# deepmarkpy/aware

Hardware: AMD Instinct MI355X
Metric: waveform-seconds/sec through embed->attack->detect; BER vs reference (higher is better)
Workload: dtype f32 accumulation on the 16-bit MFMA pipe; conv-block GEMMs: every f32 operand scaled by a power of two and carried as TWO binary16 terms (within one f32 ulp of the operand, rms 2^-24.5), 3 partial products, the l_a*l_b term (<= 2^-22) dropped -- gemm_h2.hip: error level of an f32 dot product (agains

## Files before the change

### aware_amd/_lib.py

```python
from __future__ import annotations

import ctypes as C
import glob
import os
import subprocess

_HERE = os.path.dirname(os.path.abspath(__file__))
LIB_PATH = os.environ.get("AWARE_HIP_LIB") or os.path.join(_HERE, "libaware_hip.so")
CSRC = os.path.join(_HERE, "csrc")
SOURCES = ["capi.hip", "dsp_kernels.hip", "dsp_stream.hip", "seam_kernels.hip", "detector_kernels.hip", "gemm_x3.hip", "gemm_h2.hip", "attack_kernels.hip", "stft_any.hip", "stoi_kernels.hip", "loop_attack_kernels.hip", "loop_reverb_kernels.hip", "loop_speed_kernels.hip", "loop_stretch_kernels.hip"]

AWARE_OK = 0
ERRORS = {-1: "bad argument", -2: "unsupported configuration", -3: "HIP runtime error", -4: "workspace too small"}


class AwareHipError(RuntimeError):
    pass


def build_library(force: bool = False, verbose: bool = False) -> str:
    from concurrent.futures import ThreadPoolExecutor
    hdrs = glob.glob(os.path.join(CSRC, "*.hpp")) + glob.glob(os.path.join(CSRC, "*.h")) + [
        os.path.join(_HERE, "..", "include", "aware_hip.h")]
    hdr_t = max(os.path.getmtime(h) for h in hdrs)
    bdir = os.path.join(CSRC, "build")
    os.makedirs(bdir, exist_ok=True)
    flags = ["-O3", "--offload-arch=gfx950", "-std=c++17", "-fPIC"]
    extra = {"dsp_stream.hip": ["-fno-slp-vectorize"]}
    jobs, objs = [], []
    for sname in SOURCES:
        src = os.path.join(CSRC, sname)
        obj = os.path.join(bdir, sname.replace(".hip", ".o"))
        objs.append(obj)
        if force or not os.path.exists(obj) or os.path.getmtime(obj) < max(os.path.getmtime(src), hdr_t):
            jobs.append(["hipcc"] + flags + extra.get(sname, []) + ["-c", src, "-o", obj])
    if not jobs and os.path.exists(LIB_PATH) and all(os.path.getmtime(o) <= os.path.getmtime(LIB_PATH) for o in objs):
        return LIB_PATH

    def run(cmd):
        if verbose:
            print(" ".join(cmd), flush=True)
        subprocess.run(cmd, check=True)

    with ThreadPoolExecutor(max_workers=min(6, max(1, len(jobs)))) as ex:
        list(ex.map(run, jobs))
    run(["hipcc", "--offload-arch=gfx950", "-shared", "-fPIC", "-o", LIB_PATH] + objs)
    return LIB_PATH


class EmbedConfig(C.Structure):
    _fields_ = [("num_iterations", C.c_int), ("tolerance_db", C.c_float), ("loss", C.c_int),
                ("lr", C.c_float), ("beta1", C.c_float), ("beta2", C.c_float), ("eps", C.c_float),
                ("momentum_decay", C.c_float), ("use_graph", C.c_int), ("conv_pipe", C.c_int), ("readout", C.c_int),
                ("dsp_path", C.c_int), ("l1_weight", C.c_float), ("mel", C.c_int)]


class DetectorArch(C.Structure):
    _fields_ = [("activation", C.c_int), ("norm", C.c_int), ("final_activation", C.c_int),
                ("norm_scale", C.POINTER(C.c_void_p)), ("norm_shift", C.POINTER(C.c_void_p))]


class LoopAttack(C.Structure):
    _fields_ = [("kind", C.c_int), ("param", C.c_float), ("prob", C.c_float)]


class LoopAttackEx(C.Structure):
    _fields_ = [("kind", C.c_int), ("prob", C.c_float), ("param", C.c_float * 4)]


class OptimizerConfig(C.Structure):
    _fields_ = [("kind", C.c_int), ("hyp", C.c_float * 8), ("weight_decay", C.c_double), ("table", C.POINTER(C.c_double)),
                ("plateau", C.c_int), ("patience", C.c_int), ("factor", C.c_double), ("threshold", C.c_double),
                ("min_lr", C.c_double), ("eps", C.c_double), ("lr0", C.c_double)]


_vp, _i, _f, _sz = C.c_void_p, C.c_int, C.c_float, C.c_size_t
_pi = C.POINTER(C.c_int)

SIGNATURES = {
    "aware_version": (_i, []),
    "aware_last_hip_error": (C.c_char_p, []),
    "aware_plan_create": (_i, [C.POINTER(_vp), _i, _i, _i, _i, _i, _i]),
    "aware_plan_destroy": (None, [_vp]),
    "aware_plan_create_ex": (_i, [C.POINTER(_vp), _i, _i, _i, _i, _i, _i, _i]),
    "aware_plan_spectrum_stride": (_i, [_vp]),
    "aware_plan_is_general": (_i, [_vp]),
    "aware_plan_band_stride": (_i, [_vp]),
    "aware_nola_check": (_i, [_i, _i, _i, _i, _i]),
    "aware_batch_create": (_i, [C.POINTER(_vp), _i, _pi, _pi]),
    "aware_batch_destroy": (None, [_vp]),
    "aware_batch_total_frames": (_i, [_vp]),
    "aware_batch_total_pooled": (_i, [_vp]),
    "aware_batch_total_out": (_i, [_vp]),
    "aware_batch_out_offset": (_i, [_vp, _i]),
    "aware_batch_out_length": (_i, [_vp, _i]),
    "aware_batch_frames": (_i, [_vp, _i]),
    "aware_batch_create_for_plan": (_i, [C.POINTER(_vp), _vp, _i, _pi, _pi]),
    "aware_batch_scratch_bytes": (_sz, [_vp]),
    "aware_stft": (_i, [_vp, _vp, _vp, _i, _vp, _vp, _vp]),
    "aware_istft": (_i, [_vp, _vp, _vp, _i, _vp, _vp, _vp]),
    "aware_stft_band": (_i, [_vp, _vp, _vp, _i, _vp, _vp, _vp, _vp]),
    "aware_stft_bwd": (_i, [_vp, _vp, _vp, _vp, _vp]),
    "aware_istft_bwd": (_i, [_vp, _vp, _vp, _vp, _vp]),
    "aware_detector_backward_workspace_bytes": (_sz, [_vp, _vp]),
    "aware_detector_backward": (_i, [_vp, _vp, _vp, _vp, _vp, _vp, _vp, _sz, _vp]),
    "aware_polar_decompose": (_i, [_vp, _vp, _vp, _sz, _vp]),
    "aware_polar_decompose_bwd": (_i, [_vp, _vp, _vp, _vp, _sz, _vp]),
    "aware_polar_assemble": (_i, [_vp, _vp, _vp, _sz, _vp]),
    "aware_polar_assemble_bwd": (_i, [_vp, _vp, _vp, _vp, _vp, _sz, _vp]),
    "aware_waveform_normalize_bwd": (_i, [_vp, _vp, _vp, _vp, _vp, _i, _vp]),
    "aware_nadam_coefficients": (_i, [_i, _f, _f, _f, _f, C.POINTER(C.c_float), C.POINTER(C.c_float)]),
    "aware_nadam_clamp_step": (_i, [_vp, _vp, _vp, _vp, _vp, _vp, _sz, C.POINTER(C.c_float), _f, _f, _f, _vp]),
    "aware_detector_train_workspace_bytes": (_sz, [_vp, _vp]),
    "aware_detector_weight_gradients": (_i, [_vp, _vp, _vp, _vp, _vp, _vp, C.POINTER(_vp), C.POINTER(_vp), _vp, _sz, _vp]),
    "aware_detector_update": (_i, [_vp, _vp, C.POINTER(_vp), C.POINTER(_vp)]),
    "aware_detector_train_gradients": (_i, [_vp, _vp, _vp, _vp, _i, _vp, _vp, _vp, C.POINTER(_vp), C.POINTER(_vp), _vp, _sz, _vp]),
    "aware_detector_update_device": (_i, [_vp, C.POINTER(_vp), C.POINTER(_vp), _vp]),
    "aware_detector_create": (_i, [C.POINTER(_vp), _vp, _vp, _i, _i, _pi, C.POINTER(_vp), C.POINTER(_vp)]),
    "aware_detector_create_ex": (_i, [C.POINTER(_vp), _vp, _vp, _i, _i, _pi, C.POINTER(_vp), C.POINTER(_vp),
                                     C.POINTER(DetectorArch)]),
    "aware_detector_is_card": (_i, [_vp]),
    "aware_detector_destroy": (None, [_vp]),
    "aware_detect_workspace_bytes": (_sz, [_vp, _vp]),
    "aware_detect": (_i, [_vp, _vp, _vp, _vp, _vp, _vp, _sz, _vp]),
    "aware_detector_forward": (_i, [_vp, _vp, _vp, _vp, _vp, _sz, _vp]),
    "aware_embed_workspace_bytes": (_sz, [_vp, _vp]),
    "aware_embed_create": (_i, [C.POINTER(_vp), _vp, _vp, _vp, C.POINTER(EmbedConfig), _vp, _sz, _vp]),
    "aware_embed_destroy": (None, [_vp]),
    "aware_embed_set_optimizer": (_i, [_vp, C.POINTER(OptimizerConfig), _vp]),
    "aware_embed_loop_attack_workspace_bytes": (_sz, [_vp, _i]),
    "aware_embed_set_loop_attacks": (_i, [_vp, C.POINTER(LoopAttack), _i, C.POINTER(C.c_uint32), _vp, _sz, _vp]),
    "aware_embed_loop_attack_workspace_bytes_ex": (_sz, [_vp, C.POINTER(LoopAttackEx), _i]),
    "aware_embed_set_loop_attacks_ex": (_i, [_vp, C.POINTER(LoopAttackEx), _i, C.POINTER(C.c_uint32), _vp, _sz, _vp]),
    "aware_convolve_workspace_bytes": (_sz, [_i, _i, C.c_longlong, _i]),
    "aware_convolve": (_i, [_vp, _vp, _vp, _i, _i, _vp, _i, _vp, _i, _vp, _vp, _sz, _vp]),
    "aware_reverb_ir": (_i, [_vp, _i, _i, _i, _i, _i, _f, _vp, _i, _vp, _vp]),
    "aware_speed_change": (_i, [_vp, _vp, _vp, _vp, _vp, _vp, _i, _i, _vp, _i, _vp]),
    "aware_stretch_ola": (_i, [_vp, _vp, _vp, _vp, _vp, _vp, _i, _i, _vp, _i, _vp]),
    "aware_opt_clamp_step": (_i, [_i, _vp, _vp, _vp, _vp, _vp, _vp, _sz, C.POINTER(C.c_float), C.POINTER(C.c_float), _vp]),
    "aware_embed_begin": (_i, [_vp, _vp, _vp, _vp]),
    "aware_embed_iterate": (_i, [_vp, _i, _vp]),
    "aware_embed_profile": (_i, [_vp, _i, _i, _vp, _vp, _vp]),
    "aware_embed_gradient": (_i, [_vp, _vp, _vp]),
    "aware_embed_finish": (_i, [_vp, _vp, _vp, _vp]),
    "aware_embed_buffer": (_vp, [_vp, _i]),
    "aware_pcm_quantize": (_i, [_vp, _vp, _vp, _vp, _i, _i, _i, _vp, _vp]),
    "aware_waveform_normalize": (_i, [_vp, _vp, _vp, _vp, _i, _i, _vp, _vp]),
    "aware_upfirdn": (_i, [_vp, _vp, _vp, _vp, _vp, _vp, _i, _i, _vp, _i, _i, _i, _i, _vp]),
    "aware_iir": (_i, [_vp, _vp, _vp, _i, _i, _vp, _i, _vp, _vp, _vp, _i, _i, _vp, _vp]),
    "aware_decimate_interp": (_i, [_vp, _vp, _vp, _i, _i, _i, _vp, _vp]),
    "aware_segment_cut": (_i, [_vp, _vp, _vp, _vp, _vp, _vp, _vp, _i, _i, _i, _vp]),
    "aware_phase_vocoder": (_i, [_vp, _vp, _vp, _vp, _i, C.c_double, _vp]),
    "aware_snr": (_i, [_vp, _vp, _vp, _vp, _vp, _i, _vp, _vp]),
    "aware_stoi_create": (_i, [C.POINTER(_vp)]),
    "aware_stoi_destroy": (None, [_vp]),
    "aware_stoi_band_edges": (_i, [_vp, _pi, _pi]),
    "aware_stoi_frames": (_i, [_i]),
    "aware_stoi_workspace_bytes": (_sz, [_i, _i, C.c_longlong]),
    "aware_stoi": (_i, [_vp, _vp, _vp, _vp, _vp, _vp, _i, _i, C.c_longlong, _vp, _vp, _vp, _sz, _vp]),
    "aware_gaussian_noise": (_i, [_vp, _vp, _vp, _vp, _i, _i, _vp, _f, _vp, _vp]),
    "aware_spectral_quantize": (_i, [_vp, _i, _f, _f, _vp]),
    "aware_spectral_quantize_bwd": (_i, [_vp, _vp, _vp, _i, _f, _f, _vp]),
    "aware_gemm_nt_variant": (_i, [_vp, _i, _vp, _i, _vp, _vp, _i, _i, _i, _i, _i, _vp]),
    "aware_x3_packed_bytes": (_sz, [_i, _i]),
    "aware_x3_pack": (_i, [_vp, _i, _i, _vp]),
    "aware_gemm_clip": (_i, [_vp, _i, _vp, _i, _vp, _vp, _vp, _i, _i, _i, _i, _i, _i, _vp, _vp, _i, _vp]),
    "aware_gemm_clip_last": (_i, [_vp, _i, _vp, _vp, _vp, _i, _i, _i, _i, _i, _vp, _vp, _vp, _i, _vp]),
    "aware_gemm_clip_h2_workspace_bytes": (_sz, [_i, _i, _i]),
    "aware_gemm_clip_h2": (_i, [_vp, _i, _vp, _i, _vp, _vp, _i, _i, _i, _i, _i, _i, _vp, _vp, _vp, _vp, _i, _vp, _vp, _sz, _vp]),
    "aware_gemm_nt": (_i, [_vp, _i, _vp, _i, _vp, _vp, _i, _i, _i, _i, _vp]),
}

_lib = None


def load_library():
    global _lib
    if _lib is not None:
        return _lib
    if not os.path.exists(LIB_PATH):
        raise AwareHipError(
            f"{LIB_PATH} is missing: build it with `python -c 'import __graft_entry__ as g; g.build()'` "
            "(hipcc --offload-arch=gfx950).  aware_amd has no CPU fallback.")
    import torch
    lib = C.CDLL(LIB_PATH)
    for name, (res, args) in SIGNATURES.items():
        fn = getattr(lib, name)
        fn.restype = res
        fn.argtypes = args
# ... 17 lines not shown
```

### aware_amd/csrc/capi.hip

```cpp
#include <hip/hip_runtime.h>
#include <math.h>
#include <cmath>
#include <stdio.h>
#include <stdlib.h>
#include <string.h>
#include <string>
#include <algorithm>
#include <vector>

#include "../../include/aware_hip.h"
#include "common.hpp"
#include "kernels.h"

using namespace aware;

static thread_local std::string g_last_err;

#define HIPCHK(expr)                                                                  \
    do {                                                                              \
        hipError_t _e = (expr);                                                       \
        if (_e != hipSuccess) {                                                       \
            g_last_err = std::string(#expr) + ": " + hipGetErrorString(_e);           \
            return AWARE_E_HIP;                                                       \
        }                                                                             \
// ... 1388 lines not shown
        G.tr2 = c.take<float>((size_t)b->NP * d->maxc);
    }
    if (own_loss) G.loss = c.take<float>(b->B);
    if (own_gmag) G.gmag = c.take<float>((size_t)b->NF * d->stride);
}
static size_t grad_bytes(const aware_batch* b, const aware_detector* d, bool training) {
    Carver c(nullptr, 0);
    DetBufs o;
    DetGradCtx G;
    carve_grad(c, b, d, o, G, training, !training, training);
    return c.off;
}

extern "C" size_t aware_detector_backward_workspace_bytes(const aware_batch* b, const aware_detector* d) {
    if (!b || !d) return 0;
    return grad_bytes(b, d, false);
}
extern "C" int aware_detector_backward(const aware_detector* d, const aware_batch* b, const float* mag,
                                       const float* grad_values, float* values, float* grad_mag, void* workspace,
                                       size_t workspace_bytes, void* stream) {
    if (!d || !b || b->general || !mag || !grad_values || !grad_mag || !workspace) return AWARE_E_BADARG;
    hipStream_t st = (hipStream_t)stream;
    Carver c(workspace, workspace_bytes);
    DetBufs o;
    DetGradCtx G;
    carve_grad(c, b, d, o, G, false, true, false);
    if (!c.ok) return AWARE_E_WORKSPACE;
    G.target = grad_values; G.loss_kind = AWARE_LOSS_EXTERNAL; G.gmag = grad_mag;
    int rc = det_forward_backward(d, b, det_plan(d, b, 0, 0, false, false, false), mag, o, G, st);
    if (rc) return rc;
    if (values) HIPCHK(hipMemcpyAsync(values, o.pred, (size_t)b->B * d->nbits * sizeof(float), hipMemcpyDeviceToDevice, st));
    return AWARE_OK;
}

extern "C" size_t aware_detector_train_workspace_bytes(const aware_batch* b, const aware_detector* d) {
    if (!b || !d) return 0;
    return grad_bytes(b, d, true);
}
static int detector_train_core(const aware_detector* d, const aware_batch* b, const float* mag, const float* target, int loss_kind,
                               float* loss_out, float* values, float* grad_mag, float* const* grad_weights,
                               float* const* grad_biases, void* workspace, size_t workspace_bytes, void* stream);

extern "C" int aware_detector_train_gradients(const aware_detector* d, const aware_batch* b, const float* mag, const float* target,
                                              int loss_kind, float* loss_out, float* values, float* grad_mag,
                                              float* const* grad_weights, float* const* grad_biases, void* workspace,
                                              size_t workspace_bytes, void* stream) {
    if (!d || !b || !mag || !target || !loss_out || !grad_weights || !workspace) return AWARE_E_BADARG;
    if (loss_kind < 0 || loss_kind > AWARE_LOSS_BER) return AWARE_E_BADARG;
    return detector_train_core(d, b, mag, target, loss_kind, loss_out, values, grad_mag, grad_weights, grad_biases, workspace,
                               workspace_bytes, stream);
}

extern "C" int aware_detector_weight_gradients(const aware_detector* d, const aware_batch* b, const float* mag,
                                               const float* grad_values, float* values, float* grad_mag,
                                               float* const* grad_weights, float* const* grad_biases, void* workspace,
                                               size_t workspace_bytes, void* stream) {
    if (!d || !b || !mag || !grad_values || !grad_mag || !grad_weights || !workspace) return AWARE_E_BADARG;
    return detector_train_core(d, b, mag, grad_values, AWARE_LOSS_EXTERNAL, nullptr, values, grad_mag, grad_weights, grad_biases,
                               workspace, workspace_bytes, stream);
}

static int detector_train_core(const aware_detector* d, const aware_batch* b, const float* mag, const float* target, int loss_kind,
                               float* loss_out, float* values, float* grad_mag, float* const* grad_weights,
                               float* const* grad_biases, void* workspace, size_t workspace_bytes, void* stream) {
    if (!d || !b || b->general) return AWARE_E_BADARG;
    if (!det_trainable(d)) return AWARE_E_UNSUPPORTED;
    if (d->stride != kFS) return AWARE_E_UNSUPPORTED;
    hipStream_t st = (hipStream_t)stream;
    Carver c(workspace, workspace_bytes);
    DetBufs o;
    DetGradCtx G;
    G.loss = loss_out; G.gmag = grad_mag;
    carve_grad(c, b, d, o, G, true, !loss_out, !grad_mag);
    if (!c.ok) return AWARE_E_WORKSPACE;
    HIPCHK(hipMemsetAsync(G.d1, 0, (size_t)b->NP * d->maxc * sizeof(float) * 2, st));
    G.target = target; G.loss_kind = loss_kind;
    G.wgrad = grad_weights; G.bgrad = grad_biases;
    int rc = det_forward_backward(d, b, det_plan(d, b, 1, 1, true, false, false), mag, o, G, st);
    if (rc) return rc;
    if (values) HIPCHK(hipMemcpyAsync(values, o.pred, (size_t)b->B * d->nbits * sizeof(float), hipMemcpyDeviceToDevice, st));
    return AWARE_OK;
}

struct aware_embed {
    const aware_plan* plan;
    const aware_detector* det;
    const aware_batch* b;
    aware_embed_config cfg;
    DetBufs db;
    float *coef, *lo, *hi, *mom, *vel, *best, *mag, *gmag;
    cf *P, *U;
    float *yraw, *oob, *gy;
    float* gpad;
    float* c0 = nullptr;
    double* pl1 = nullptr;
    float* l1term = nullptr;
    float *d1, *d2;
    float *loss, *best_loss, *target;
    int *improved, *step;
    float4* sched;
    unsigned long long *pmaxA, *pmaxY;
    double* pdot;
    float hyp[4];
    hipGraph_t graph = nullptr, graphN = nullptr;
    hipGraphExec_t gexec = nullptr, gexecN = nullptr;
    hipStream_t cap = nullptr;
    int steps_done = 0;
    struct {
        bool active = false;
        int kind = 0, plateau = 0, patience = 0;
        float hyp[8] = {0};
        double wd = 0, factor = 0, threshold = 0, min_lr = 0, eps = 0, lr0 = 0;
        double* d_tab = nullptr;
        double* d_lr = nullptr;
        double* d_state = nullptr;
        std::vector<double> lr_init, state_init;
    } opt;
    struct {
        int n = 0;
        int kind[kMaxLoopAttacks] = {0}, k[kMaxLoopAttacks] = {0};
        double inv_snr[kMaxLoopAttacks] = {0};
        float prob[kMaxLoopAttacks] = {0};
        float* z = nullptr;
        unsigned long long* pmaxZ = nullptr;
        double* psq = nullptr;
        double* pdot = nullptr;
        float* gpad0 = nullptr;
        unsigned* seeds = nullptr;
        int rv = -1, n_lo = 0, n_hi = 0, kmax = 0;
        double gain = 0;
        float* u = nullptr;
        float* h = nullptr;
        int* nh = nullptr;
        cf* tables = nullptr;
        cf* hspec = nullptr;
        cf* xspec = nullptr;
        int sp = -1, m_lo = 0, m_hi = 0;
        int ts = -1, q_lo = 0, q_hi = 0;
        float* v = nullptr;
        const float* hann = nullptr;
        bool locked = false;
    } la;
};

static void carve_embed(Carver& c, const aware_batch* b, const aware_detector* det, int iters, bool l1, aware_embed* e) {
    carve_det(c, b, det, e->db);
    const size_t nsp = (size_t)b->NF * det->stride;
    e->coef = c.take<float>(nsp); e->lo = c.take<float>(nsp); e->hi = c.take<float>(nsp);
    e->mom = c.take<float>(nsp); e->vel = c.take<float>(nsp); e->best = c.take<float>(nsp);
    e->mag = c.take<float>(nsp); e->gmag = c.take<float>(nsp);
    e->P = c.take<cf>(nsp); e->U = c.take<cf>(nsp);
    e->yraw = c.take<float>(b->NS); e->oob = c.take<float>(b->NS); e->gy = c.take<float>(b->NS);
    e->gpad = c.take<float>((size_t)b->B * 1024);
    e->d1 = c.take<float>((size_t)b->NP * det->maxc); e->d2 = c.take<float>((size_t)b->NP * det->maxc);
    e->loss = c.take<float>(b->B); e->best_loss = c.take<float>(b->B);
    e->target = c.take<float>((size_t)b->B * det->nbits);
    e->improved = c.take<int>(b->B); e->step = c.take<int>(4);
    e->sched = c.take<float4>(iters + 1);
    e->pmaxA = c.take<unsigned long long>((size_t)b->B * b->pstride);
    e->pmaxY = c.take<unsigned long long>((size_t)b->B * b->pstride);
    e->pdot = c.take<double>((size_t)b->B * b->pstride);
    e->c0 = c.take<float>(nsp);
    e->opt.d_tab = c.take<double>((size_t)iters * 5);
    e->opt.d_lr = c.take<double>(b->B);
    e->opt.d_state = c.take<double>((size_t)b->B * 3);
    if (l1) {
        e->pl1 = c.take<double>((size_t)b->B * b->pstride);
        e->l1term = c.take<float>(b->B);
    }
}
extern "C" size_t aware_embed_workspace_bytes(const aware_batch* b, const aware_detector* d) {
    if (!b || !d) return 0;
    Carver c(nullptr, 0);
    aware_embed e;
    carve_embed(c, b, d, 4096, true, &e);
    return c.off;
}

static void nadam_coefficients(int s, double lr, double b1, double b2, double md, float& mu_product, float out[3]) {
    const double bc2 = 1.0 - pow(b2, (double)s);
    const double mu = b1 * (1.0 - 0.5 * pow(0.96, s * md));
    const double mu_next = b1 * (1.0 - 0.5 * pow(0.96, (s + 1) * md));
    mu_product = mu_product * (float)mu;
    const double mp = (double)mu_product;
    out[0] = (float)(-lr * (1.0 - mu) / (1.0 - mp));
    out[1] = (float)((-lr * mu_next) / (1.0 - mp * mu_next));
    out[2] = (float)bc2;
}
extern "C" int aware_nadam_coefficients(int step, float lr, float beta1, float beta2, float momentum_decay,
                                        float* mu_product_io, float* coef3) {
    if (step < 1 || !mu_product_io || !coef3) return AWARE_E_BADARG;
    nadam_coefficients(step, lr, beta1, beta2, momentum_decay, *mu_product_io, coef3);
    return AWARE_OK;
}
extern "C" int aware_nadam_clamp_step(float* param, const float* grad, float* exp_avg, float* exp_avg_sq, const float* lo,
                                      const float* hi, size_t n, const float* coef3, float beta1, float beta2, float eps,
                                      void* stream) {
    if (!param || !grad || !exp_avg || !exp_avg_sq || !coef3 || n < 1) return AWARE_E_BADARG;
    launch_nadam_clamp(param, grad, exp_avg, exp_avg_sq, lo, hi, n, coef3[0], coef3[1], coef3[2], beta1, beta2, eps,
                       (hipStream_t)stream);
    LAUNCHCHK();
    return AWARE_OK;
}
extern "C" int aware_opt_clamp_step(int kind, float* param, const float* grad, float* state1, float* state2, const float* lo,
                                    const float* hi, size_t n, const float* coef4, const float* hyp8, void* stream) {
    if (kind < 0 || kind > 7 || !param || !grad || !state1 || !state2 || !coef4 || !hyp8 || n < 1) return AWARE_E_BADARG;
    launch_opt_clamp(kind, param, grad, state1, state2, lo, hi, n, coef4, hyp8, (hipStream_t)stream);
    LAUNCHCHK();
    return AWARE_OK;
}
extern "C" int aware_waveform_normalize_bwd(const float* in, const float* grad_out, float* grad_in, const int* off,
                                            const int* len, int B, void* stream) {
    if (!in || !grad_out || !grad_in || !off || !len || B < 1) return AWARE_E_BADARG;
    launch_normalize_bwd(in, grad_out, grad_in, off, len, B, (hipStream_t)stream);
    LAUNCHCHK();
    return AWARE_OK;
}
extern "C" int aware_polar_decompose(const void* spec, float* mag, float* phase, size_t n, void* stream) {
    if (!spec || !mag || n < 1) return AWARE_E_BADARG;
    launch_polar_decompose(spec, mag, phase, n, (hipStream_t)stream);
    LAUNCHCHK();
    return AWARE_OK;
}
extern "C" int aware_polar_decompose_bwd(const void* spec, const float* grad_mag, const float* grad_phase, void* grad_spec,
                                         size_t n, void* stream) {
    if (!spec || !grad_spec || (!grad_mag && !grad_phase) || n < 1) return AWARE_E_BADARG;
    launch_polar_decompose_bwd(spec, grad_mag, grad_phase, grad_spec, n, (hipStream_t)stream);
    LAUNCHCHK();
    return AWARE_OK;
}
extern "C" int aware_polar_assemble(const float* mag, const float* phase, void* spec, size_t n, void* stream) {
    if (!mag || !phase || !spec || n < 1) return AWARE_E_BADARG;
    launch_polar_assemble(mag, phase, spec, n, (hipStream_t)stream);
    LAUNCHCHK();
    return AWARE_OK;
}
extern "C" int aware_polar_assemble_bwd(const float* mag, const float* phase, const void* grad_spec, float* grad_mag,
                                        float* grad_phase, size_t n, void* stream) {
    if (!mag || !phase || !grad_spec || (!grad_mag && !grad_phase) || n < 1) return AWARE_E_BADARG;
    launch_polar_assemble_bwd(mag, phase, grad_spec, grad_mag, grad_phase, n, (hipStream_t)stream);
    LAUNCHCHK();
    return AWARE_OK;
}

extern "C" int aware_embed_create(aware_embed** out, const aware_plan* plan, const aware_detector* det,
                                  const aware_batch* b, const aware_embed_config* cfg, void* workspace,
                                  size_t workspace_bytes, void* stream) {
    if (!out || !plan || !det || !b || !cfg || !workspace) return AWARE_E_BADARG;
    if (plan->general) return AWARE_E_UNSUPPORTED;
    if (b->general) return AWARE_E_BADARG;
    if (cfg->num_iterations < 1 || cfg->num_iterations > 4096 || cfg->loss < 0 || cfg->loss > AWARE_LOSS_PUSH_L1) return AWARE_E_BADARG;
    if (cfg->conv_pipe < 0 || cfg->conv_pipe > 2 || cfg->readout < 0 || cfg->readout > 1 || cfg->mel < 0 || cfg->mel > 1)
        return AWARE_E_BADARG;
    if (cfg->dsp_path < 0 || cfg->dsp_path > 1) return AWARE_E_BADARG;
    if (det->band_lo != plan->dev.band_lo || det->nband != plan->dev.nband || det->stride != plan->dev.stride) return AWARE_E_BADARG;
    const bool l1 = cfg->loss == AWARE_LOSS_PUSH_L1;
    if (l1 && (cfg->dsp_path != 0 || !stream_supported(plan->dev))) return AWARE_E_UNSUPPORTED;
    hipStream_t st = (hipStream_t)stream;
    aware_embed* e = new aware_embed();
    e->plan = plan; e->det = det; e->b = b; e->cfg = *cfg;
    Carver c(workspace, workspace_bytes);
    carve_embed(c, b, det, cfg->num_iterations, l1, e);
    if (!c.ok) { delete e; return AWARE_E_WORKSPACE; }
    const size_t nsp = (size_t)b->NF * plan->dev.stride;
    HIPCHK(hipMemsetAsync(e->mag, 0, nsp * sizeof(float), st));
    HIPCHK(hipMemsetAsync(e->U, 0, nsp * sizeof(cf), st));
    HIPCHK(hipMemsetAsync(e->gpad, 0, (size_t)b->B * 1024 * sizeof(float), st));
    std::vector<float4> sc(cfg->num_iterations + 1);
    float mu_product = 1.0f;
    const double b1 = cfg->beta1, b2 = cfg->beta2;
    for (int s = 1; s <= cfg->num_iterations; ++s) {
        float c3[3];
        nadam_coefficients(s, cfg->lr, b1, b2, cfg->momentum_decay, mu_product, c3);
        sc[s - 1] = make_float4(c3[0], c3[1], c3[2], 0.f);
    }
    sc[cfg->num_iterations] = sc[cfg->num_iterations - 1];
    HIPCHK(hipMemcpyAsync(e->sched, sc.data(), sc.size() * sizeof(float4), hipMemcpyHostToDevice, st));
    HIPCHK(hipStreamSynchronize(st));
    e->hyp[0] = (float)(1.0 - b1); e->hyp[1] = (float)b2; e->hyp[2] = (float)(1.0 - b2); e->hyp[3] = cfg->eps;
    {
        HIPCHK(hipMemsetAsync(e->d1, 0, (size_t)b->NP * det->maxc * sizeof(float), st));
        HIPCHK(hipMemsetAsync(e->mag, 0, nsp * sizeof(float), st));
        auto f32_shape = [&](int M, int N, int K, int lda) {
            return !(cfg->conv_pipe != 1 && M % 32 == 0 && gemm_clip_x3_supported(1, N, K, lda));
        };
        const int S = det->stride;
        const int Mp = det->ch[0];
        if (f32_shape(b->NF, Mp, S, S)) gemm_autotune(e->mag, S, det->melT, S, e->db.xm, Mp, b->NF, Mp, S, st);
        if (f32_shape(b->NF, S, Mp, Mp)) gemm_autotune(e->db.xm, Mp, det->melB, Mp, e->gmag, S, b->NF, S, Mp, st);
        for (int l = 0; l < det->n_layers; ++l) {
            const int ci = det->ch[l], co = det->ch[l + 1];
            if (f32_shape(b->NP, co, ci, ci)) gemm_autotune(e->d1, ci, det->w[l], ci, e->d2, co, b->NP, co, ci, st);
            if (f32_shape(b->NP, ci, co, co)) gemm_autotune(e->d1, co, det->wT[l], co, e->d2, ci, b->NP, ci, co, st);
        }
        HIPCHK(hipStreamSynchronize(st));
    }
    *out = e;
    return AWARE_OK;
}
extern "C" int aware_embed_set_optimizer(aware_embed* e, const aware_optimizer_config* oc, void* stream) {
    if (!e || !oc || oc->kind < 0 || oc->kind > 7 || !oc->table) return AWARE_E_BADARG;
    if (e->gexec) return AWARE_E_BADARG;
    if (oc->plateau && (!(oc->factor < 1.0) || oc->patience < 0)) return AWARE_E_BADARG;
// ... 178 lines not shown
                              int h_stride, const int* nh, int adjoint, float* out, void* workspace, size_t workspace_bytes,
                              void* stream) {
    if (!in || !off || !len || !h || !nh || !out || !workspace || ((uintptr_t)workspace & 255)) return AWARE_E_BADARG;
    if (B < 1 || B > 65535 || max_len < 1 || h_stride < 1 || h_stride > kReverbMaxIr || adjoint < 0 || adjoint > 1)
        return AWARE_E_BADARG;
    ConvolveLaunch L;
    L.B = B; L.kmax = reverb_blocks(max_len); L.parts = convolve_parts(h_stride);
    Carver c(workspace, workspace_bytes);
    carve_convolve(c, B, L.kmax, L.parts, L);
    if (!c.ok) return AWARE_E_WORKSPACE;
    hipStream_t st = (hipStream_t)stream;
    const std::vector<cf>& t = reverb_tables();
    HIPCHK(hipMemcpyAsync(const_cast<cf*>(L.tables), t.data(), t.size() * sizeof(cf), hipMemcpyHostToDevice, st));
    L.in = in; L.out = out; L.off = off; L.len = len; L.h = h; L.h_stride = h_stride; L.nh = nh; L.adjoint = adjoint;
    launch_convolve(L, st);
    LAUNCHCHK();
    return AWARE_OK;
}
extern "C" int aware_reverb_ir(const uint32_t* seeds, int B, int step, int entry, int n_lo, int n_hi, float drr_db, float* h,
                               int h_stride, int* nh, void* stream) {
    if (!seeds || !h || !nh || B < 1 || B > 65535 || step < 0 || entry < 0 || entry >= kMaxLoopAttacks) return AWARE_E_BADARG;
    if (n_lo < 2 || n_hi > kReverbMaxIr || n_lo > n_hi || h_stride < n_hi || !std::isfinite(drr_db)) return AWARE_E_BADARG;
    ReverbIrLaunch L;
    L.seeds = seeds; L.step_imm = step; L.entry = entry; L.B = B; L.n_lo = n_lo; L.n_hi = n_hi;
    L.gain = pow(10.0, (double)drr_db / 20.0); L.prob = 1.f; L.h = h; L.h_stride = h_stride; L.nh = nh;
    launch_reverb_ir(L, (hipStream_t)stream);
    LAUNCHCHK();
    return AWARE_OK;
}

extern "C" int aware_speed_change(const float* in, const int* in_off, const int* in_len, float* out, const int* out_off,
                                  const int* out_len, int B, int max_len, const int* m, int adjoint, void* stream) {
    if (!in || !in_off || !in_len || !out || !out_off || !out_len || !m || in == out) return AWARE_E_BADARG;
    if (B < 1 || B > 65535 || max_len < 1 || max_len > (1 << 30) || adjoint < 0 || adjoint > 1) return AWARE_E_BADARG;
    SpeedLaunch L;
    L.in = in; L.out = out; L.B = B; L.adjoint = adjoint; L.max_len = max_len; L.m = m;
    L.x_off = in_off; L.x_len = in_len; L.z_off = out_off; L.z_len = out_len;
    launch_speed_change(L, (hipStream_t)stream);
    LAUNCHCHK();
    return AWARE_OK;
}

extern "C" int aware_stretch_ola(const float* in, const int* in_off, const int* in_len, float* out, const int* out_off,
                                 const int* out_len, int B, int max_len, const int* m, int adjoint, void* stream) {
    if (!in || !in_off || !in_len || !out || !out_off || !out_len || !m || in == out) return AWARE_E_BADARG;
    if (B < 1 || B > 65535 || max_len < 1 || max_len > (1 << 30) || adjoint < 0 || adjoint > 1) return AWARE_E_BADARG;
    StretchLaunch L;
    if (!(L.window = stretch_window())) return AWARE_E_HIP;
    L.in = in; L.out = out; L.B = B; L.adjoint = adjoint; L.max_len = max_len; L.m = m;
    L.x_off = in_off; L.x_len = in_len; L.z_off = out_off; L.z_len = out_len;
    launch_time_stretch(L, (hipStream_t)stream);
    LAUNCHCHK();
    return AWARE_OK;
}

extern "C" void aware_embed_destroy(aware_embed* e) {
    if (!e) return;

    if (e->gexec) (void)hipGraphExecDestroy(e->gexec);
    if (e->graph) (void)hipGraphDestroy(e->graph);
    if (e->gexecN) (void)hipGraphExecDestroy(e->gexecN);
    if (e->graphN) (void)hipGraphDestroy(e->graphN);
    if (e->cap) (void)hipStreamDestroy(e->cap);
    delete e;
}

extern "C" void* aware_embed_buffer(aware_embed* e, int which) {
    if (!e) return nullptr;
    switch (which) {
        case 0: return e->loss;
        case 1: return e->best_loss;
        case 2: return e->db.pred;
        case 3: return e->coef;
        case 4: return e->best;
        case 5: return e->lo;
        case 6: return e->hi;
        case 7: return e->P;
        case 8: return e->step;
        case 9: return e->yraw;
        case 10: return e->mag;
        case 11: return e->opt.active ? e->opt.d_lr : nullptr;
        case 12: return e->la.n ? e->la.z : nullptr;
        case 13: return (e->la.n && e->la.rv >= 0) ? e->la.h : nullptr;
        default: return nullptr;
    }
}

extern "C" int aware_embed_begin(aware_embed* e, const float* audio, const float* target, void* stream) {
    if (!e || !audio || !target) return AWARE_E_BADARG;
    hipStream_t st = (hipStream_t)stream;
    const aware_batch* b = e->b;
    launch_absmax_partials(audio, b->d_in_off, b->d_in_len, e->pmaxA, b->pstride, b->B, b->max_len, st);
    LAUNCHCHK();
    AnalysisLaunch L;
    L.plan = e->plan->dev; L.frame_off = b->d_frame_off; L.B = b->B; L.max_frames = b->max_frames; L.run_frames = b->an_run; L.wg_tab = b->d_an_wg; L.n_wg = b->n_an_wg;
    L.sig = audio; L.sig_off = b->d_in_off; L.sig_len = b->d_in_len;
    L.pmax = e->pmaxA; L.pcount = b->d_pc_in; L.pstride = b->pstride;
    L.mag = e->mag; L.unit = e->P; L.unit_default = 1.f;
    run_analysis(L, e->cfg.dsp_path, st);
    LAUNCHCHK();
    SynthLaunch S;
    S.plan = e->plan->dev; S.frame_off = b->d_frame_off; S.B = b->B; S.max_frames = b->max_frames; S.run_blocks = b->synth_run; S.wg_tab = b->d_syn_wg; S.n_wg = b->n_syn_wg;
    S.amp = e->mag; S.ph = e->P; S.out = e->gy; S.pstride = b->pstride;
    run_synth(S, e->cfg.dsp_path, st);
    LAUNCHCHK();
    launch_oob_residual(audio, b->d_in_off, e->pmaxA, b->d_pc_in, b->pstride, e->gy, b->d_frame_off, e->oob, b->B,
                        b->max_frames, st);
    LAUNCHCHK();
    const float ratio = (float)pow(10.0, -(double)e->cfg.tolerance_db / 20.0);
    launch_embed_prepare(e->mag, e->coef, e->lo, e->hi, e->mom, e->vel, e->best, e->c0, ratio, (size_t)b->NF * e->plan->dev.stride, st);
    LAUNCHCHK();
    HIPCHK(hipMemcpyAsync(e->target, target, (size_t)b->B * e->det->nbits * sizeof(float), hipMemcpyDeviceToDevice, st));
    HIPCHK(hipMemsetAsync(e->step, 0, 4 * sizeof(int), st));
    HIPCHK(hipMemsetD32Async((hipDeviceptr_t)e->best_loss, 0x7F800000, b->B, st));
    if (e->opt.active) {
        HIPCHK(hipMemcpyAsync(e->opt.d_lr, e->opt.lr_init.data(), (size_t)b->B * sizeof(double), hipMemcpyHostToDevice, st));
        HIPCHK(hipMemcpyAsync(e->opt.d_state, e->opt.state_init.data(), (size_t)b->B * 3 * sizeof(double), hipMemcpyHostToDevice, st));
    }
    e->steps_done = 0;
    return AWARE_OK;
}

static SpeedLaunch speed_launch(const aware_embed* e, const float* in, float* out, int adjoint, int step_back) {
    const auto& la = e->la;
    SpeedLaunch S;
    S.in = in; S.out = out; S.B = e->b->B; S.adjoint = adjoint; S.frame_off = e->b->d_frame_off; S.pstride = e->b->pstride;
    S.run_blocks = e->b->synth_run; S.step = e->step; S.step_back = step_back; S.seeds = la.seeds; S.entry = la.sp;
    S.m_lo = la.m_lo; S.m_hi = la.m_hi; S.prob = la.prob[la.sp];
    return S;
}

static StretchLaunch stretch_launch(const aware_embed* e, const float* in, float* out, int adjoint, int step_back) {
    const auto& la = e->la;
    StretchLaunch S;
    S.in = in; S.out = out; S.window = la.hann; S.B = e->b->B; S.adjoint = adjoint; S.frame_off = e->b->d_frame_off;
    S.pstride = e->b->pstride; S.run_blocks = e->b->synth_run; S.step = e->step; S.step_back = step_back; S.seeds = la.seeds;
    S.entry = la.ts; S.m_lo = la.q_lo; S.m_hi = la.q_hi; S.prob = la.prob[la.ts];
    return S;
}

static ConvolveLaunch reverb_launch(const aware_embed* e, const float* in, float* out, int adjoint) {
    const auto& la = e->la;
    ConvolveLaunch C;
    C.tables = la.tables; C.in = in; C.out = out; C.frame_off = e->b->d_frame_off; C.B = e->b->B; C.kmax = la.kmax;
    C.h = la.h; C.h_stride = kReverbMaxIr; C.nh = la.nh; C.parts = kReverbParts; C.adjoint = adjoint; C.skip_h = adjoint;
    C.hspec = la.hspec; C.xspec = la.xspec;
    return C;
}

static int embed_iteration(aware_embed* e, hipStream_t st, int do_step, float* grad_out) {
    const aware_batch* b = e->b;
    const aware_detector* d = e->det;
    SynthLaunch S;
    S.plan = e->plan->dev; S.frame_off = b->d_frame_off; S.B = b->B; S.max_frames = b->max_frames; S.run_blocks = b->synth_run; S.wg_tab = b->d_syn_wg; S.n_wg = b->n_syn_wg;
    S.amp = e->coef; S.ph = e->P; S.out = e->yraw; S.add = e->oob; S.pmax = e->pmaxY; S.pstride = b->pstride;
    S.c0 = e->pl1 ? e->c0 : nullptr; S.pl1 = e->pl1;
    const int dsp = e->cfg.dsp_path;
    run_synth(S, dsp, st);
    LAUNCHCHK(); PROF(K_SYNTH);
    if (e->pl1) {
        launch_l1_reduce(e->pl1, b->d_pc_syn, b->pstride, b->d_frame_off, e->plan->dev.nband, e->cfg.l1_weight, e->l1term, b->B, st);
        LAUNCHCHK(); PROF(K_MISC);
    }
    AnalysisLaunch L;
    L.plan = e->plan->dev; L.frame_off = b->d_frame_off; L.B = b->B; L.max_frames = b->max_frames; L.run_frames = b->an_run; L.wg_tab = b->d_an_wg; L.n_wg = b->n_an_wg;
    L.sig = e->yraw; L.sig_off = b->d_out_off; L.sig_len = b->d_out_len;
    L.pmax = e->pmaxY; L.pcount = b->d_pc_syn; L.pstride = b->pstride; L.double_norm = 1;
    const bool attacked = e->la.n > 0;
    LoopAttackLaunch A;
    if (attacked) {
        const auto& la = e->la;
        A.frame_off = b->d_frame_off; A.pcount = b->d_pc_syn; A.B = b->B; A.pstride = b->pstride; A.run_blocks = b->synth_run;
        A.step = e->step; A.seeds = la.seeds; A.n = la.n;
        for (int j = 0; j < la.n; ++j) { A.kind[j] = la.kind[j]; A.k[j] = la.k[j]; A.inv_snr[j] = la.inv_snr[j]; A.prob[j] = la.prob[j]; }
        A.yraw = e->yraw; A.pmaxY = e->pmaxY; A.psq = la.psq; A.z = la.z; A.pmaxZ = la.pmaxZ;
        if (la.rv >= 0 || la.sp >= 0 || la.ts >= 0) { A.idle_plain = 1; A.gpad_out = la.gpad0; }
        if (la.ts >= 0) {
            const bool pair = la.sp >= 0;
            launch_loop_attack_stage(A, 0, la.ts, e->yraw, 1, la.u, nullptr, st);
            launch_time_stretch(stretch_launch(e, la.u, pair ? la.v : la.z, 0, 0), st);
            if (pair) launch_speed_change(speed_launch(e, la.v, la.z, 0, 0), st);
            launch_loop_attack_stage(A, (pair ? la.sp : la.ts) + 1, la.n, la.z, 0, la.z, la.pmaxZ, st);
        } else if (la.sp >= 0) {
            launch_loop_attack_stage(A, 0, la.sp, e->yraw, 1, la.u, nullptr, st);
            launch_speed_change(speed_launch(e, la.u, la.z, 0, 0), st);
            launch_loop_attack_stage(A, la.sp + 1, la.n, la.z, 0, la.z, la.pmaxZ, st);
        } else if (la.rv < 0) {
            launch_loop_attack_forward(A, st);
        } else {
            launch_loop_attack_stage(A, 0, la.rv, e->yraw, 1, la.u, nullptr, st);
            ReverbIrLaunch R;
            R.seeds = la.seeds; R.step = e->step; R.entry = la.rv; R.B = b->B; R.n_lo = la.n_lo; R.n_hi = la.n_hi;
            R.gain = la.gain; R.prob = la.prob[la.rv]; R.h = la.h; R.h_stride = kReverbMaxIr; R.nh = la.nh;
            launch_reverb_ir(R, st);
            launch_convolve(reverb_launch(e, la.u, la.z, 0), st);
            launch_loop_attack_stage(A, la.rv + 1, la.n, la.z, 0, la.z, la.pmaxZ, st);
        }
        LAUNCHCHK(); PROF(K_MISC);
        L.sig = la.z; L.pmax = la.pmaxZ;
    }
    L.mag = e->mag; L.unit = e->U; L.unit_default = 0.f; L.write_pad = 0;
    const bool mel_taps = dsp == 0 && d->n_mels == 128 && d->melw && d->melm && stream_supported(e->plan->dev) && e->cfg.mel == 0;
    const bool mel_fold = mel_taps && d->melf_w && d->melf_s && d->n_mels == 128;
    if (mel_fold) { L.mel_out = e->db.xm; L.melf_w = d->melf_w; L.melf_s = d->melf_s; }
    run_analysis(L, dsp, st);
    LAUNCHCHK(); PROF(K_ANALYSIS);
    DetGradCtx G;
    G.target = e->target; G.loss_kind = e->cfg.loss;
    G.loss = e->loss; G.d1 = e->d1; G.d2 = e->d2; G.gmag = e->gmag; G.loss_add = e->l1term;
    G.step = do_step ? e->step : nullptr;
    G.best_loss = do_step ? e->best_loss : nullptr;
    G.improved = do_step ? e->improved : nullptr;
    const DetPlan p = det_plan(d, b, e->cfg.conv_pipe, e->cfg.readout, false, mel_fold, mel_taps);
    int rc = det_forward_backward(d, b, p, e->mag, e->db, G, st);
    if (rc) return rc;
    SynthLaunch SA;
    SA.plan = e->plan->dev; SA.frame_off = b->d_frame_off; SA.B = b->B; SA.max_frames = b->max_frames; SA.run_blocks = b->synth_run; SA.wg_tab = b->d_syn_wg; SA.n_wg = b->n_syn_wg;
    SA.amp = e->gmag; SA.ph = e->U; SA.out = e->gy; SA.adjoint = 1; SA.yraw = e->yraw; SA.pmax_in = e->pmaxY;
    SA.pcount = b->d_pc_syn; SA.pdot = e->pdot; SA.pstride = b->pstride; SA.gpad = e->gpad;
    if (mel_taps) { SA.dmel = e->db.xm; SA.melw = d->melw; SA.melm = d->melm; }
    if (attacked) { SA.yraw = e->la.z; SA.pmax_in = e->la.pmaxZ; }
    run_synth(SA, dsp, st);
    LAUNCHCHK(); PROF(K_SYNTH_ADJ);
    if (attacked) {
        const bool streamed = dsp == 0 && stream_supported(e->plan->dev);
        A.step_back = do_step ? 1 : 0;
        A.gy = e->gy; A.gpad = streamed ? e->gpad : nullptr; A.pdot_in = e->pdot; A.pdot_out = e->la.pdot;
        if (e->la.ts >= 0) {
            const bool pair = e->la.sp >= 0;
            A.gy_out = e->la.u;
            launch_loop_attack_stage_bwd(A, (pair ? e->la.sp : e->la.ts) + 1, e->la.n, 1, 0, st);
            A.gy_out = nullptr;
            if (pair) launch_speed_change(speed_launch(e, e->la.u, e->la.v, 1, A.step_back), st);
            launch_time_stretch(stretch_launch(e, pair ? e->la.v : e->la.u, e->gy, 1, A.step_back), st);
            launch_loop_attack_stage_bwd(A, 0, e->la.ts, 0, 1, st);
        } else if (e->la.sp >= 0) {
            A.gy_out = e->la.u;
            launch_loop_attack_stage_bwd(A, e->la.sp + 1, e->la.n, 1, 0, st);
            A.gy_out = nullptr;
            launch_speed_change(speed_launch(e, e->la.u, e->gy, 1, A.step_back), st);
            launch_loop_attack_stage_bwd(A, 0, e->la.sp, 0, 1, st);
        } else if (e->la.rv < 0) {
            launch_loop_attack_backward(A, st);
        } else {
            launch_loop_attack_stage_bwd(A, e->la.rv + 1, e->la.n, 1, 0, st);
            launch_convolve(reverb_launch(e, e->gy, e->gy, 1), st);
            launch_loop_attack_stage_bwd(A, 0, e->la.rv, 0, 1, st);
        }
        LAUNCHCHK(); PROF(K_MISC);
    }
    AnalysisLaunch LA;
    LA.plan = e->plan->dev; LA.frame_off = b->d_frame_off; LA.B = b->B; LA.max_frames = b->max_frames; LA.run_frames = b->an_run; LA.wg_tab = b->d_an_wg; LA.n_wg = b->n_an_wg;
    LA.sig = e->gy; LA.sig_off = b->d_out_off; LA.sig_len = b->d_out_len;
    LA.pmax = e->pmaxY; LA.pcount = b->d_pc_syn; LA.pstride = b->pstride;
    LA.adjoint = 1; LA.yraw = e->yraw; LA.pdot = e->pdot; LA.phasor = e->P;
    LA.coef = e->coef; LA.mom = e->mom; LA.vel = e->vel; LA.lo = e->lo; LA.hi = e->hi; LA.best = e->best;
    LA.improved = e->improved; LA.sched = e->sched; LA.sched_len = e->cfg.num_iterations + 1; LA.step = e->step;
    const bool own_step = do_step && e->opt.active;
    LA.grad_out = own_step ? e->gmag : grad_out; LA.do_step = own_step ? 0 : do_step;
    memcpy(LA.hyp, e->hyp, sizeof(LA.hyp));
    LA.gpad = e->gpad; LA.c0 = e->c0; LA.box_ratio = (float)pow(10.0, -(double)e->cfg.tolerance_db / 20.0);
    LA.l1_weight = e->pl1 ? e->cfg.l1_weight : 0.f;
    if (attacked) { LA.pdot = e->la.pdot; LA.gpad = e->la.gpad0; }
    run_analysis(LA, dsp, st);
    LAUNCHCHK(); PROF(K_ANALYSIS_ADJ);
    if (own_step) {
        const auto& o = e->opt;
        launch_opt_rows(o.kind, e->coef, e->gmag, e->mom, e->vel, e->c0, LA.box_ratio, e->best, e->improved, b->d_frame_off, b->B,
                        b->NF, o.d_tab, e->cfg.num_iterations, e->step, o.plateau ? o.d_lr : nullptr, o.wd, o.hyp,
                        e->plan->dev.nband, e->plan->dev.stride, st);
        if (o.plateau)
            launch_plateau(e->loss, o.d_state, o.d_lr, b->B, o.factor, o.patience, o.threshold, o.min_lr, o.eps, st);
        LAUNCHCHK(); PROF(K_MISC);
    }
    return AWARE_OK;
}

extern "C" int aware_embed_iterate(aware_embed* e, int n_iters, void* stream) {
    if (!e || n_iters < 0) return AWARE_E_BADARG;
    if (e->steps_done + n_iters > e->cfg.num_iterations) return AWARE_E_BADARG;
    hipStream_t st = (hipStream_t)stream;
    if (n_iters > 0) e->la.locked = true;
    if (!e->cfg.use_graph) {
        for (int i = 0; i < n_iters; ++i) {
            int rc = embed_iteration(e, st, 1, nullptr);
            if (rc) return rc;
            ++e->steps_done;
        }
        return AWARE_OK;
    }
    constexpr int kGraphIters = 16;
    if (!e->gexec) {
        if (!e->cap) HIPCHK(hipStreamCreateWithFlags(&e->cap, hipStreamNonBlocking));
        for (int which = 0; which < 2; ++which) {
            HIPCHK(hipStreamBeginCapture(e->cap, hipStreamCaptureModeThreadLocal));
            int rc = AWARE_OK;
            for (int i = 0; i < (which ? kGraphIters : 1) && rc == AWARE_OK; ++i) rc = embed_iteration(e, e->cap, 1, nullptr);
            hipGraph_t g = nullptr;
            hipError_t ce = hipStreamEndCapture(e->cap, &g);
            hipGraphExec_t ge = nullptr;
            if (rc == AWARE_OK && ce == hipSuccess) ce = hipGraphInstantiate(&ge, g, nullptr, nullptr, 0);
            if (rc != AWARE_OK || ce != hipSuccess) {
                if (ge) (void)hipGraphExecDestroy(ge);
                if (g) (void)hipGraphDestroy(g);
                if (e->gexec) { (void)hipGraphExecDestroy(e->gexec); e->gexec = nullptr; }
                if (e->graph) { (void)hipGraphDestroy(e->graph); e->graph = nullptr; }
                if (rc != AWARE_OK) return rc;
                HIPCHK(ce);
            }
            if (which) { e->graphN = g; e->gexecN = ge; } else { e->graph = g; e->gexec = ge; }
        }
    }
    int left = n_iters;
    for (; left >= kGraphIters; left -= kGraphIters) { HIPCHK(hipGraphLaunch(e->gexecN, st)); e->steps_done += kGraphIters; }
    for (; left > 0; --left) { HIPCHK(hipGraphLaunch(e->gexec, st)); ++e->steps_done; }
    return AWARE_OK;
}

extern "C" int aware_embed_profile(aware_embed* e, int n_iters, int max_entries, float* ms_out, int* kind_out,
                                   void* stream) {
    if (!e || !ms_out || !kind_out || n_iters < 1) return AWARE_E_BADARG;
    if (e->steps_done + n_iters > e->cfg.num_iterations) return AWARE_E_BADARG;
    hipStream_t st = (hipStream_t)stream;
    LaunchProfiler p;
    p.st = st;
    g_prof = &p;
    prof_mark(-1);
    int rc = AWARE_OK;
    for (int i = 0; i < n_iters && rc == AWARE_OK; ++i) { rc = embed_iteration(e, st, 1, nullptr); if (rc == AWARE_OK) ++e->steps_done; }
    g_prof = nullptr;
    hipError_t se = hipStreamSynchronize(st);
    int n = 0;
    for (size_t i = 1; i < p.ev.size(); ++i) {
        float ms = 0.f;
        (void)hipEventElapsedTime(&ms, p.ev[i - 1], p.ev[i]);
        if (n < max_entries) { ms_out[n] = ms; kind_out[n] = p.kind[i]; ++n; }
    }
    for (auto& ev : p.ev) (void)hipEventDestroy(ev);
    if (rc) return rc;
    HIPCHK(se);
    return n;
}

extern "C" int aware_embed_gradient(aware_embed* e, float* grad, void* stream) {
    if (!e || !grad) return AWARE_E_BADARG;
    return embed_iteration(e, (hipStream_t)stream, 0, grad);
}

extern "C" int aware_embed_finish(aware_embed* e, const float* rescale, float* out, void* stream) {
    if (!e || !out) return AWARE_E_BADARG;
    hipStream_t st = (hipStream_t)stream;
    const aware_batch* b = e->b;
    SynthLaunch S;
    S.plan = e->plan->dev; S.frame_off = b->d_frame_off; S.B = b->B; S.max_frames = b->max_frames; S.run_blocks = b->synth_run; S.wg_tab = b->d_syn_wg; S.n_wg = b->n_syn_wg;
    S.amp = e->best; S.ph = e->P; S.out = e->yraw; S.add = e->oob; S.pmax = e->pmaxY; S.pstride = b->pstride;
    run_synth(S, e->cfg.dsp_path, st);
    LAUNCHCHK();
    launch_finish(e->yraw, b->d_frame_off, e->pmaxY, b->d_pc_syn, b->pstride, rescale, out, b->d_out_off, b->B,
                  b->max_frames, st);
    LAUNCHCHK();
    return AWARE_OK;
}

extern "C" int aware_pcm_quantize(const float* in, float* out, const int* off, const int* len, int B, int max_len,
                                  int bits, void* scratch, void* stream) {
    if (!in || !out || !off || !len || !scratch || B < 1) return AWARE_E_BADARG;
    float q, lo, hi;
    switch (bits) {
        case 8: q = 127.f; lo = -128.f; hi = 127.f; break;
        case 12: q = 4095.f; lo = -4096.f; hi = 4095.f; break;
        case 16: q = 32767.f; lo = -32768.f; hi = 32767.f; break;
        case 24: q = 8388607.f; lo = -8388608.f; hi = 8388607.f; break;
        default: return AWARE_E_BADARG;
    }
    hipStream_t st = (hipStream_t)stream;
    unsigned long long* pmax; int* pcount; int ps;
    int rc = absmax_into_scratch(in, off, len, B, max_len, scratch, &pmax, &pcount, &ps, st);
    if (rc) return rc;
    launch_pcm_quantize(in, out, off, len, pmax, pcount, ps, q, lo, hi, B, max_len, st);
    LAUNCHCHK();
    return AWARE_OK;
}

static int absmax_into_scratch(const float* in, const int* off, const int* len, int B, int max_len, void* scratch,
                               unsigned long long** pmax_out, int** pcount_out, int* ps_out, hipStream_t st) {
    const int ps = (max_len + 4095) / 4096;
    unsigned long long* pmax = (unsigned long long*)scratch;
    int* pcount = (int*)(pmax + (size_t)B * ps);
    HIPCHK(hipMemsetAsync(pmax, 0, (size_t)B * ps * sizeof(unsigned long long), st));
    launch_absmax_partials(in, off, len, pmax, ps, B, max_len, st);
    LAUNCHCHK();
    HIPCHK(hipMemsetD32Async((hipDeviceptr_t)pcount, ps, B, st));
    *pmax_out = pmax; *pcount_out = pcount; *ps_out = ps;
    return AWARE_OK;
}

extern "C" int aware_waveform_normalize(const float* in, float* out, const int* off, const int* len, int B,
                                        int max_len, void* scratch, void* stream) {
    if (!in || !out || !off || !len || !scratch || B < 1) return AWARE_E_BADARG;
    hipStream_t st = (hipStream_t)stream;
    unsigned long long* pmax; int* pcount; int ps;
    int rc = absmax_into_scratch(in, off, len, B, max_len, scratch, &pmax, &pcount, &ps, st);
    if (rc) return rc;
    launch_normalize(in, out, off, len, pmax, pcount, ps, B, max_len, st);
    LAUNCHCHK();
    return AWARE_OK;
}

extern "C" int aware_upfirdn(const float* in, const int* in_off, const int* in_len, float* out, const int* out_off,
                             const int* out_len, int B, int max_out, const float* h, int nh, int up, int down,
                             int half_len, void* stream) {
    if (!in || !out || !h || B < 1 || up < 1 || down < 1) return AWARE_E_BADARG;
    launch_upfirdn(in, in_off, in_len, out, out_off, out_len, h, nh, up, down, half_len, B, max_out,
// ... 294 lines not shown
```

### aware_amd/csrc/dsp_args.hpp

```cpp
#pragma once
#include "common.hpp"

namespace aware {

#ifndef AWARE_EXACT_DIV
__device__ __forceinline__ float fast_rcp(float x) { return __builtin_amdgcn_rcpf(x); }
__device__ __forceinline__ float fast_sqrt(float x) { return __builtin_amdgcn_sqrtf(x); }
#else
__device__ __forceinline__ float fast_rcp(float x) { return 1.0f / x; }
__device__ __forceinline__ float fast_sqrt(float x) { return sqrtf(x); }
#endif

__device__ __forceinline__ void nadam_clamp_update(float& p, float& mo, float& ve, float g, float blo, float bhi,
                                                   float c_grad, float c_mom, float inv_bc2, const float4& hyp) {
    mo = mo + hyp.x * (g - mo);
    ve = ve * hyp.y + (hyp.z * g) * g;
    const float rden = fast_rcp(fast_sqrt(ve * inv_bc2) + hyp.w);
    p = p + (c_grad * g) * rden;
    p = p + (c_mom * mo) * rden;
    p = fminf(fmaxf(p, blo), bhi);
}

enum { OPT_NADAM = 0, OPT_ADAM = 1, OPT_ADAMW = 2, OPT_SGD = 3, OPT_RMSPROP = 4, OPT_ADAGRAD = 5, OPT_ADAMAX = 6, OPT_ADADELTA = 7 };
struct OptHyp { float h[8]; };
__device__ __forceinline__ void opt_clamp_update(int kind, float& p, float& mo, float& ve, float g, float blo, float bhi,
                                                 const float4& c, const OptHyp& H) {
    const float* h = H.h;
    if (h[7] != 0.f) g = g * h[7];
    if (kind == OPT_ADAMW) p = p * c.w;
    else if (h[4] != 0.f) g = g + h[4] * p;
    if (kind == OPT_NADAM) {
        mo = mo + h[0] * (g - mo);
        ve = ve * h[1] + (h[2] * g) * g;
        const float den = sqrtf(ve / c.z) + h[3];
        p = p + (c.x * g) / den;
        p = p + (c.y * mo) / den;
    } else if (kind == OPT_ADAM || kind == OPT_ADAMW) {
        mo = mo + h[0] * (g - mo);
        ve = ve * h[1] + (h[2] * g) * g;
        const float den = sqrtf(ve) / c.z + h[3];
        p = p + (c.x * mo) / den;
    } else if (kind == OPT_SGD) {
        float d = g;
        if (h[0] != 0.f) {
            mo = (c.y != 0.f) ? g : mo * h[0] + h[6] * g;
            d = (h[5] != 0.f) ? g + h[0] * mo : mo;
        }
        p = p + c.x * d;
    } else if (kind == OPT_RMSPROP) {
        ve = ve * h[1] + (h[2] * g) * g;
        const float avg = sqrtf(ve) + h[3];
        if (h[0] != 0.f) {
            mo = mo * h[0] + g / avg;
            p = p + c.x * mo;
        } else p = p + (c.x * g) / avg;
    } else if (kind == OPT_ADAGRAD) {
        ve = ve + g * g;
        const float sd = sqrtf(ve) + h[3];
        p = p + (c.x * g) / sd;
    } else if (kind == OPT_ADAMAX) {
        mo = mo + h[0] * (g - mo);
        ve = fmaxf(ve * h[1], fabsf(g) + h[3]);
        p = p + (c.x * mo) / ve;
    } else {
        ve = ve * h[1] + (h[2] * g) * g;
        const float sd = sqrtf(ve + h[3]);
        const float delta = sqrtf(mo + h[3]) / sd * g;
        mo = mo * h[1] + (h[2] * delta) * delta;
        p = p + c.x * delta;
    }
    p = fminf(fmaxf(p, blo), bhi);
}

__device__ __forceinline__ void box_bounds(float c0, float ratio, float& lo, float& hi) {
    const float d = __fmul_rn(c0, ratio);
    lo = fmaxf(__fsub_rn(c0, d), 0.f);
    hi = __fadd_rn(c0, d);
}

enum { AN_NORM = 0, AN_ADJ = 1 };
enum { SY_FWD = 0, SY_ADJ = 1 };

struct AnalysisArgs {
    PlanDev plan;
    const int* frame_off;
    const int* wg_tab;
    const float* sig;
    const int* sig_off;
    const int* sig_len;
    const unsigned long long* pmax;
    const int* pcount;
    int pstride;
    int double_norm;
    float unit_default;
    float* mag;
    cf* unit;
    cf* full;
    const float* yraw;
    const double* pdot;
    const cf* phasor;
    float* coef;
    float* mom;
    float* vel;
    const float* lo;
    const float* hi;
    float* best;
    const int* improved;
    const float4* sched;
    int sched_len;
    const int* step;
    float* grad_out;
    int do_step;
    float4 hyp;
    const float* gpad;
    int write_pad;
    const float* c0;
    float box_ratio;
    float l1_weight;
    float* mel_out;
    const float* melf_w;
    const unsigned char* melf_s;
};



struct SynthArgs {
    PlanDev plan;
    const int* frame_off;
    const int* wg_tab;
    const float* amp;
    const cf* ph;
    const cf* full;
    float* out;
    const float* add;
    unsigned long long* pmax;
    int pstride;
    const float* yraw;
    const unsigned long long* pmax_in;
    const int* pcount;
    double* pdot;
    float* gpad;
    int run_blocks;
    const float* c0;
    double* pl1;
    const int* sig_off;
    const int* sig_len;
    const float* dmel;
    const float2* melw;
    const unsigned char* melm;
};


}
```

### aware_amd/csrc/dsp_kernels.hip

```cpp
#include "common.hpp"
#include "dsp_args.hpp"
#include "kernels.h"

namespace aware {

__global__ __launch_bounds__(kThreads) void absmax_partial_kernel(const float* __restrict__ sig,
                                                                   const int* __restrict__ sig_off,
                                                                   const int* __restrict__ sig_len,
                                                                   unsigned long long* __restrict__ pmax,
                                                                   int pstride) {
    __shared__ unsigned long long red[4];
    const int b = blockIdx.y;
    const int n = sig_len[b];
    const int s0 = blockIdx.x * 4096;
    if (s0 >= n) return;
    const float* x = sig + sig_off[b];
    unsigned long long v = 0;
    for (int i = s0 + threadIdx.x; i < min(n, s0 + 4096); i += kThreads) v = umax64(v, pack_max(fabsf(x[i]), i));
    v = wave_max64(v);
    if ((threadIdx.x & 63) == 0) red[threadIdx.x >> 6] = v;
    __syncthreads();
    if (threadIdx.x == 0) pmax[(size_t)b * pstride + blockIdx.x] = umax64(umax64(red[0], red[1]), umax64(red[2], red[3]));
}

// ... 14 lines not shown
    const int n = a.sig_len[b];
    const float* x = a.sig + a.sig_off[b];
    const int tid = threadIdx.x;

    float m = 1.f, m2 = 1.f;
    unsigned kmax = 0xFFFFFFFFu;
    if (a.pmax) {
        ClipNorm cn = clip_norm_from_partials(a.pmax + (size_t)b * a.pstride, a.pcount[b], red);
        m = cn.m;
        m2 = (MODE == AN_ADJ || a.double_norm) ? cn.m2 : 1.f;
        kmax = cn.k;
    }
    float adot = 0.f, smax = 0.f;
    if (MODE == AN_ADJ && a.pdot) {
        double s = 0.0;
        const double* pd = a.pdot + (size_t)b * a.pstride;
        for (int i = tid; i < a.pcount[b]; i += kThreads) s += pd[i];
        s = wave_sum_d(s);
        if ((tid & 63) == 0) dred[tid >> 6] = s;
        __syncthreads();
        adot = (float)(dred[0] + dred[1] + dred[2] + dred[3]);
        float yk = a.yraw[a.sig_off[b] + kmax];
        smax = (yk > 0.f) ? 1.f : ((yk < 0.f) ? -1.f : 0.f);
    }

    const int p0 = kHop * t0;
    const int cnt = kHop * (nfr - 1) + kNfft;
    {
        constexpr int NIT = kChunk / kThreads;
        const bool small_t = T < 4;
        const float inv_m = 1.0f / m, inv_m2 = 1.0f / m2, inv_mm2 = 1.0f / (m * m2);
        float xin[NIT], env[NIT];
#pragma unroll
        for (int it = 0; it < NIT; ++it) {
            const int p = p0 + tid + kThreads * it;
            int src = p - kHalf;
            if (MODE == AN_NORM) {
                if (src < 0) src = -src;
                if (src >= n) src = 2 * (n - 1) - src;
            }
            xin[it] = x[min(max(src, 0), n - 1)];
            if (MODE == AN_ADJ) env[it] = small_t ? 1.f : a.plan.env_tab[ola_envelope_index(p, T)];
        }
#pragma unroll
        for (int it = 0; it < NIT; ++it) {
            const int i = tid + kThreads * it;
            if (i < cnt) {
                const int p = p0 + i;
                const int src = p - kHalf;
                float v;
                if (MODE == AN_NORM) {
                    v = xin[it];
                    if (a.pmax) { v = v * inv_m; if (a.double_norm) v = v * inv_m2; }
                } else {
                    if (src >= 0 && src < n) {
                        float g = xin[it];
                        if ((unsigned)src == kmax) g -= adot * smax;
                        g = g * inv_mm2;
                        v = g * fast_rcp(small_t ? ola_envelope_loop(a.plan.window2, p, T) : env[it]);
                    } else {
                        v = 0.f;
                    }
                }
                chunk[i] = v;
            }
        }
    }
    __syncthreads();

    const int wave = __builtin_amdgcn_readfirstlane(tid >> 6), lane = tid & 63;
    cf* s = scratch[wave];
    FftLaneConst fc;
    fft_lane_const(lane, a.plan.tw512, fc);
    float wr[16];
#pragma unroll
    for (int r = 0; r < 8; ++r) {
        wr[2 * r] = a.plan.window[2 * (lane + 64 * r)];
        wr[2 * r + 1] = a.plan.window[2 * (lane + 64 * r) + 1];
    }
    const int band_lo = a.plan.band_lo, nband = a.plan.nband;
    const int S = a.plan.stride;
    float4 sc = make_float4(0.f, 0.f, 1.f, 0.f);
    float inv_bc2 = 1.f;
    int improved = 0;
    if (MODE == AN_ADJ && a.do_step) {
        sc = a.sched[min(max(*a.step - 1, 0), a.sched_len - 1)];
        inv_bc2 = 1.0f / sc.z;
        improved = a.improved[b];
    }

    const bool pre_ok = (MODE == AN_ADJ) && a.do_step && band_lo < 64;
#pragma unroll 1
    for (int fr = wave; fr < nfr; fr += 4) {
        cf v[8];
        const size_t row = (size_t)(f0 + t0 + fr);
        cf preP[5];
        float preM[5], preV[5], preC[5], preL[5], preH[5];
        if (MODE == AN_ADJ) {
#pragma unroll
            for (int r = 0; r < 5; ++r) {
                const int f = lane + 64 * r - band_lo;
                preP[r] = mk(0.f, 0.f); preM[r] = preV[r] = preC[r] = preL[r] = preH[r] = 0.f;
                if (pre_ok && f >= 0 && f < nband) {
                    const size_t idx = row * S + f;
                    preP[r] = a.phasor[idx]; preM[r] = a.mom[idx]; preV[r] = a.vel[idx]; preC[r] = a.coef[idx];
                    preL[r] = a.lo[idx]; preH[r] = a.hi[idx];
                }
            }
        }
        const float2* c2 = reinterpret_cast<const float2*>(chunk + kHop * fr);
#pragma unroll
        for (int r = 0; r < 8; ++r) {
            float2 q = c2[lane + 64 * r];
            v[r] = mk(q.x * wr[2 * r], q.y * wr[2 * r + 1]);
        }
        fft512_wave<-1>(lane, v, fc, s);
        rfft_split_store(lane, v, s);
        wave_sync();
        if (FULLOUT) {
            cf* out = a.full + row * 520;
            const float si = (MODE == AN_ADJ) ? (1.0f / 512.0f) : 1.0f, se = (MODE == AN_ADJ) ? (1.0f / 1024.0f) : 1.0f;
#pragma unroll
            for (int r = 0; r < 8; ++r) {
                const int k = lane + 64 * r;
                cf X = rfft_split_bin(k, v[r], s, a.plan.tw1024);
                const float sk = k == 0 ? se : si;
                X = mk(X.x * sk, (MODE == AN_ADJ && k == 0) ? 0.f : X.y * sk);
                out[k] = X;
            }
            if (lane == 0) out[512] = mk(rfft_split_nyquist(s) * se, 0.f);
        }
        if (!FULLOUT) {
#pragma unroll
            for (int r = 0; r < 9; ++r) {
                if (r == 8 && (lane != 0 || band_lo + nband != 513)) continue;
                const int k = lane + 64 * r;
                const int f = k - band_lo;
                if (f < 0 || f >= S) continue;
                const size_t idx = row * S + f;
                if (f >= nband) {
                    if (MODE == AN_NORM) {
                        if (a.mag) a.mag[idx] = 0.f;
                        if (a.unit) a.unit[idx] = mk(0.f, 0.f);
                    }
                    continue;
                }
                cf X = (r < 8) ? rfft_split_bin(k, v[r < 8 ? r : 0], s, a.plan.tw1024) : mk(rfft_split_nyquist(s), 0.f);
                if (MODE == AN_NORM) {
                    const float mg = fast_sqrt(X.x * X.x + X.y * X.y);
                    const float im = fast_rcp(mg);
                    if (a.mag) a.mag[idx] = mg;
                    if (a.unit) a.unit[idx] = (mg > 0.f) ? mk(X.x * im, X.y * im) : mk(a.unit_default, 0.f);
                } else {
                    const bool pre = pre_ok && r < 5;
                    cf P = pre ? preP[r < 5 ? r : 0] : a.phasor[idx];
                    float g = (X.x * P.x + X.y * P.y) * (1.0f / 512.0f);
                    if (k == 0 || k == 512) g = (X.x * P.x) * (1.0f / 1024.0f);
                    if (a.grad_out) a.grad_out[idx] = g;
                    if (a.do_step) {
                        float mo, ve, p, blo, bhi;
                        if (pre) { mo = preM[r < 5 ? r : 0]; ve = preV[r < 5 ? r : 0]; p = preC[r < 5 ? r : 0];
                                   blo = preL[r < 5 ? r : 0]; bhi = preH[r < 5 ? r : 0]; }
                        else { mo = a.mom[idx]; ve = a.vel[idx]; p = a.coef[idx]; blo = a.lo[idx]; bhi = a.hi[idx]; }
                        nadam_clamp_update(p, mo, ve, g, blo, bhi, sc.x, sc.y, inv_bc2, a.hyp);
                        a.mom[idx] = mo; a.vel[idx] = ve; a.coef[idx] = p;
                        if (improved) a.best[idx] = p;
                    }
                }
            }
            if (MODE == AN_NORM && S > kFS)
                for (int f = max(nband, 512 - band_lo) + lane; f < S; f += 64) {
                    const size_t idx = row * S + f;
                    if (a.mag) a.mag[idx] = 0.f;
                    if (a.unit) a.unit[idx] = mk(0.f, 0.f);
                }
        }
        wave_sync();
    }
}


template <int MODE, int INP>
__global__ __launch_bounds__(kThreads) void synth_kernel(SynthArgs a) {
    __shared__ float ola[kSynthChunk];
    __shared__ cf scratch[4][kFftScratch];
    __shared__ unsigned long long red[4];
    __shared__ double dred[4];

    const int b = blockIdx.y;
    const int f0 = a.frame_off[b];
    const int T = a.frame_off[b + 1] - f0;
    const int nblk = T - 1;
    int nseg, jb0, jb1;
    synth_segment(nblk, blockIdx.x, a.run_blocks, nseg, jb0, jb1);
    if ((int)blockIdx.x >= nseg || T < 1) return;
    const int tid = threadIdx.x;
    const int wave = __builtin_amdgcn_readfirstlane(tid >> 6), lane = tid & 63;

    int tlo = max(0, jb0 - 1);
    int thi = min(T - 1, jb1 + 1);
    if (MODE == SY_ADJ) {
        if (blockIdx.x == 0) tlo = 0;
        if ((int)blockIdx.x == nseg - 1) thi = T - 1;
    }
    const int nfr = thi - tlo + 1;
    const int pbase = kHop * tlo;

    ClipNorm cn;
    cn.m = 1.f; cn.m2 = 1.f; cn.k = 0;
    if (MODE == SY_ADJ && a.pmax_in) cn = clip_norm_from_partials(a.pmax_in + (size_t)b * a.pstride, a.pcount[b], red);

    __shared__ cf tw1s[512];
    __shared__ cf tw2s[64];
    fft_fill_tables(tid, kThreads, a.plan.tw512, tw1s, tw2s);
    for (int i = tid; i < kSynthChunk; i += kThreads) ola[i] = 0.f;
    __syncthreads();

    cf* s = scratch[wave];
    const float scale = (MODE == SY_FWD) ? (1.0f / 512.0f) : 1.0f;
    const float2* win2p = reinterpret_cast<const float2*>(a.plan.window);
    const int band_lo = a.plan.band_lo, nband = a.plan.nband;

    constexpr bool full_in = (INP == 0);
    constexpr bool compact = (INP == 1);
    float inA[8];
    cf inP[8];
    auto load_band = [&](int fi) {
        const size_t row = (size_t)(f0 + tlo + fi);
        const float* A = a.amp + row * kFS;
        const cf* P = a.ph + row * kFS;
#pragma unroll
        for (int r = 0; r < 8; ++r) {
            const int k = lane + 64 * r;
            const int f = ((k <= 256) ? k : 512 - k) - band_lo;
            const int fc_ = min(max(f, 0), kFS - 1);
            const float am = A[fc_];
            inP[r] = P[fc_];
            inA[r] = (f >= 0 && f < nband) ? am : 0.f;
        }
    };
    cf mc[8];
    if (compact) {
#pragma unroll
        for (int r = 0; r < 8; ++r) {
            const cf w = a.plan.tw1024[lane + 64 * r];
            mc[r] = (r < 4) ? mk(0.5f * (1.f + w.y), 0.5f * w.x) : mk(0.5f * (1.f - w.y), -0.5f * w.x);
        }
    }
    if (compact && kSynthRounds * wave < nfr) load_band(kSynthRounds * wave);
// ... 100 lines not shown
        const float* y = a.yraw ? a.yraw + sig_offset(a.frame_off, b) : nullptr;
        const float inv_m = 1.0f / cn.m, inv_m2 = 1.0f / cn.m2;
        double acc = 0.0;
        float yv[NOUT];
#pragma unroll
        for (int it = 0; it < NOUT; ++it) {
            const int j = j0 + tid + kThreads * it;
            yv[it] = y ? y[j < j1 ? j : j0] : 0.f;
        }
#pragma unroll
        for (int it = 0; it < NOUT; ++it) {
            const int j = j0 + tid + kThreads * it;
            if (j < j1) {
                float g = ola[kHalf + j - pbase];
                if (j >= 1 && j <= kHalf) g += ola[kHalf - j - pbase];
                if (j >= Ny - kHalf - 1 && j <= Ny - 2) g += ola[2 * Ny + kHalf - 2 - j - pbase];
                out[j] = g;
                float y2 = (yv[it] * inv_m) * inv_m2;
                acc += (double)g * (double)y2;
            }
        }
        acc = wave_sum_d(acc);
        if (lane == 0) dred[wave] = acc;
        __syncthreads();
        if (tid == 0 && a.pdot) a.pdot[(size_t)b * a.pstride + blockIdx.x] = dred[0] + dred[1] + dred[2] + dred[3];
    }
}

__global__ void embed_prepare_kernel(const float* __restrict__ c0, float* __restrict__ coef, float* __restrict__ lo,
                                     float* __restrict__ hi, float* __restrict__ mom, float* __restrict__ vel,
                                     float* __restrict__ best, float* __restrict__ c0_keep, float ratio, size_t n) {
    size_t i = (size_t)blockIdx.x * blockDim.x + threadIdx.x;
    if (i >= n) return;
    float c = c0[i];
    coef[i] = c;
    box_bounds(c, ratio, lo[i], hi[i]);
    if (c0_keep) c0_keep[i] = c;
    mom[i] = 0.f;
    vel[i] = 0.f;
    best[i] = c;
}

__global__ void oob_residual_kernel(const float* __restrict__ audio, const int* __restrict__ in_off,
                                    const unsigned long long* __restrict__ pmax, const int* __restrict__ pcount, int pstride,
                                    const float* __restrict__ band, const int* __restrict__ frame_off, float* __restrict__ oob) {
    __shared__ unsigned long long red[4];
    const int b = blockIdx.y;
    ClipNorm cn = clip_norm_from_partials(pmax + (size_t)b * pstride, pcount[b], red);
    const int Ny = kHop * (frame_off[b + 1] - frame_off[b] - 1);
    const int so = sig_offset(frame_off, b);
    const float* x = audio + in_off[b];
    for (int j = blockIdx.x * blockDim.x + threadIdx.x; j < Ny; j += gridDim.x * blockDim.x)
        oob[so + j] = x[j] / cn.m - band[so + j];
}

__global__ void finish_kernel(const float* __restrict__ yraw, const int* __restrict__ frame_off,
                              const unsigned long long* __restrict__ pmax, const int* __restrict__ pcount, int pstride,
                              const float* __restrict__ rescale, float* __restrict__ out, const int* __restrict__ out_off) {
    __shared__ unsigned long long red[4];
    const int b = blockIdx.y;
    ClipNorm cn = clip_norm_from_partials(pmax + (size_t)b * pstride, pcount[b], red);
    const int Ny = kHop * (frame_off[b + 1] - frame_off[b] - 1);
    const int so = sig_offset(frame_off, b);
    const float r = rescale ? rescale[b] : 1.f;
    for (int j = blockIdx.x * blockDim.x + threadIdx.x; j < Ny; j += gridDim.x * blockDim.x)
        out[out_off[b] + j] = r * (yraw[so + j] / cn.m);
}

static inline dim3 grid2(int x, int y) { return dim3((unsigned)x, (unsigned)y, 1); }

void launch_absmax_partials(const float* sig, const int* sig_off, const int* sig_len, unsigned long long* pmax,
                            int pstride, int B, int max_len, hipStream_t st) {
    int nx = (max_len + 4095) / 4096;
    hipLaunchKernelGGL(absmax_partial_kernel, grid2(nx, B), dim3(kThreads), 0, st, sig, sig_off, sig_len, pmax, pstride);
}

void launch_analysis(const AnalysisLaunch& L, hipStream_t st) {
    AnalysisArgs a{};
    a.plan = L.plan;
    a.frame_off = L.frame_off;
    a.sig = L.sig; a.sig_off = L.sig_off; a.sig_len = L.sig_len;
    a.pmax = L.pmax; a.pcount = L.pcount; a.pstride = L.pstride;
    a.double_norm = L.double_norm; a.unit_default = L.unit_default;
    a.mag = L.mag; a.unit = (cf*)L.unit; a.full = (cf*)L.full;
    a.yraw = L.yraw; a.pdot = L.pdot; a.phasor = (const cf*)L.phasor;
    a.coef = L.coef; a.mom = L.mom; a.vel = L.vel; a.lo = L.lo; a.hi = L.hi; a.best = L.best;
    a.improved = L.improved; a.sched = (const float4*)L.sched; a.sched_len = L.sched_len > 0 ? L.sched_len : 1; a.step = L.step;
    a.grad_out = L.grad_out; a.do_step = L.do_step;
    a.hyp = make_float4(L.hyp[0], L.hyp[1], L.hyp[2], L.hyp[3]);
    int nx = (L.max_frames + kFramesPerWG - 1) / kFramesPerWG;
    if (L.adjoint && L.full)
        hipLaunchKernelGGL((analysis_kernel<AN_ADJ, true>), grid2(nx, L.B), dim3(kThreads), 0, st, a);
    else if (L.adjoint)
        hipLaunchKernelGGL((analysis_kernel<AN_ADJ, false>), grid2(nx, L.B), dim3(kThreads), 0, st, a);
    else if (L.full)
        hipLaunchKernelGGL((analysis_kernel<AN_NORM, true>), grid2(nx, L.B), dim3(kThreads), 0, st, a);
    else
        hipLaunchKernelGGL((analysis_kernel<AN_NORM, false>), grid2(nx, L.B), dim3(kThreads), 0, st, a);
}

void launch_synth(const SynthLaunch& L, hipStream_t st) {
    SynthArgs a{};
    a.plan = L.plan;
    a.frame_off = L.frame_off;
    a.amp = L.amp; a.ph = (const cf*)L.ph; a.full = (const cf*)L.full;
    a.out = L.out; a.add = L.add; a.pmax = L.pmax; a.pstride = L.pstride;
    a.yraw = L.yraw; a.pmax_in = L.pmax_in; a.pcount = L.pcount; a.pdot = L.pdot;
    a.sig_off = L.sig_off; a.sig_len = L.sig_len;
    int nblk = L.max_frames - 1;
    a.run_blocks = (L.run_blocks >= 1 && L.run_blocks <= kSynthBlocks) ? L.run_blocks : kSynthBlocks;
    int nx = (nblk + a.run_blocks - 1) / a.run_blocks;
    if (nx < 1) nx = 1;
    const bool compact = L.plan.band_lo >= 1 && L.plan.band_lo + L.plan.nband <= 257;
    if (L.adjoint && L.full) {
        hipLaunchKernelGGL((synth_kernel<SY_ADJ, 0>), grid2(nx, L.B), dim3(kThreads), 0, st, a);
    } else if (L.adjoint) {
        if (compact) hipLaunchKernelGGL((synth_kernel<SY_ADJ, 1>), grid2(nx, L.B), dim3(kThreads), 0, st, a);
        else hipLaunchKernelGGL((synth_kernel<SY_ADJ, 2>), grid2(nx, L.B), dim3(kThreads), 0, st, a);
    } else if (L.full) {
        hipLaunchKernelGGL((synth_kernel<SY_FWD, 0>), grid2(nx, L.B), dim3(kThreads), 0, st, a);
    } else {
        if (compact) hipLaunchKernelGGL((synth_kernel<SY_FWD, 1>), grid2(nx, L.B), dim3(kThreads), 0, st, a);
        else hipLaunchKernelGGL((synth_kernel<SY_FWD, 2>), grid2(nx, L.B), dim3(kThreads), 0, st, a);
    }
}

void launch_embed_prepare(const float* c0, float* coef, float* lo, float* hi, float* mom, float* vel, float* best,
                          float* c0_keep, float ratio, size_t n, hipStream_t st) {
    hipLaunchKernelGGL(embed_prepare_kernel, dim3((unsigned)((n + 255) / 256)), dim3(256), 0, st, c0, coef, lo, hi, mom,
                       vel, best, c0_keep, ratio, n);
}

void launch_oob_residual(const float* audio, const int* in_off, const unsigned long long* pmax, const int* pcount,
                         int pstride, const float* band, const int* frame_off, float* oob, int B, int max_frames,
                         hipStream_t st) {
    int nx = max(1, (kHop * (max_frames - 1) + 1023) / 1024);
    hipLaunchKernelGGL(oob_residual_kernel, grid2(nx, B), dim3(256), 0, st, audio, in_off, pmax, pcount, pstride, band,
                       frame_off, oob);
}

void launch_finish(const float* yraw, const int* frame_off, const unsigned long long* pmax, const int* pcount,
                   int pstride, const float* rescale, float* out, const int* out_off, int B, int max_frames,
                   hipStream_t st) {
    int nx = max(1, (kHop * (max_frames - 1) + 1023) / 1024);
    hipLaunchKernelGGL(finish_kernel, grid2(nx, B), dim3(256), 0, st, yraw, frame_off, pmax, pcount, pstride, rescale,
                       out, out_off);
}

}
```

### aware_amd/csrc/dsp_stream.hip

```cpp
#include "common.hpp"
#include "dsp_args.hpp"
#include "kernels.h"

namespace aware {

constexpr int kSW = kStreamWaves;
constexpr int kSThreads = 64 * kSW;

__device__ __forceinline__ ClipNorm clip_norm_wave(const unsigned long long* part, int nseg, int lane) {
    unsigned long long v = 0;
    for (int i = lane; i < nseg; i += 64) v = umax64(v, part[i]);
    v = wave_max64(v);
    ClipNorm c;
    const float raw = __uint_as_float((unsigned)(v >> 32));
    c.k = 0xFFFFFFFFu - (unsigned)(v & 0xFFFFFFFFu);
    c.m = raw + 1e-8f;
    c.m2 = raw / c.m + 1e-8f;
    return c;
}
__device__ __forceinline__ double dot_wave(const double* part, int nseg, int lane) {
    double s = 0.0;
    for (int i = lane; i < nseg; i += 64) s += part[i];
    return wave_sum_d(s);
}
// ... 40 lines not shown

    float m = 1.f, m2 = 1.f;
    unsigned kmax = 0xFFFFFFFFu;
    if (a.pmax) {
        const ClipNorm cn = clip_norm_wave(a.pmax + (size_t)b * a.pstride, a.pcount[b], lane);
        m = cn.m;
        m2 = (MODE == AN_ADJ || a.double_norm) ? cn.m2 : 1.f;
        kmax = cn.k;
    }
    const float inv_m = 1.0f / m, inv_m2 = 1.0f / m2, inv_mm2 = 1.0f / (m * m2);
    float corr = 0.f;
    const float* gpL = nullptr;
    const float* gpR = nullptr;
    LaneEnv le;
    le.lo = le.hi = make_float2(1.f, 1.f);
    if (MODE == AN_ADJ) {
        const float adot = (float)dot_wave(a.pdot + (size_t)b * a.pstride, a.pcount[b], lane);
        const float yk = a.yraw[a.sig_off[b] + kmax];
        corr = adot * ((yk > 0.f) ? 1.f : ((yk < 0.f) ? -1.f : 0.f));
        gpL = a.gpad + (size_t)b * 1024;
        gpR = gpL + 512;
        le = lane_env(a.plan, lane);
    }

    auto load_half = [&](int P) -> float2 {
        const int s_lo = P - kHalf;
        float2 v;
        if (MODE == AN_NORM) {
            if (al8 && s_lo >= 0 && s_lo + 128 <= n) {
                v = *reinterpret_cast<const float2*>(x + s_lo + 2 * lane);
            } else {
                int s0 = s_lo + 2 * lane, s1 = s0 + 1;
                s0 = s0 < 0 ? -s0 : s0;
                s1 = s1 < 0 ? -s1 : s1;
                s0 = s0 >= n ? 2 * (n - 1) - s0 : s0;
                s1 = s1 >= n ? 2 * (n - 1) - s1 : s1;
                v.x = x[min(max(s0, 0), n - 1)];
                v.y = x[min(max(s1, 0), n - 1)];
            }
            if (a.pmax) {
                v.x = v.x * inv_m;
                v.y = v.y * inv_m;
                if (a.double_norm) { v.x = v.x * inv_m2; v.y = v.y * inv_m2; }
            }
            return v;
        }
        if (al8 && T >= 4 && s_lo >= 513 && s_lo + 127 <= n - 514 && P >= 768 && P + 127 < kHop * T) {
            float2 g = *reinterpret_cast<const float2*>(x + s_lo + 2 * lane);
            const unsigned s = (unsigned)(s_lo + 2 * lane);
            if (s == kmax) g.x -= corr;
            if (s + 1 == kmax) g.y -= corr;
            g.x = g.x * inv_mm2;
            g.y = g.y * inv_mm2;
            const float2 re = (P & 128) ? le.hi : le.lo;
            return make_float2(g.x * re.x, g.y * re.y);
        }
        float o[2];
#pragma unroll
        for (int e = 0; e < 2; ++e) {
            const int p = P + 2 * lane + e;
            const int src = p - kHalf;
            const bool valid = src >= 0 && src < n;
            float g = x[min(max(src, 0), n - 1)];
            const bool cl = src >= 1 && src <= kHalf;
            const bool cr = src >= n - kHalf - 1 && src <= n - 2;
            const float pl = gpL[min(max(kHalf - src, 0), 511)];
            const float pr = gpR[min(max(n - 2 - src, 0), 511)];
            if (cl) g += pl;
            if (cr) g += pr;
            if ((unsigned)src == kmax) g -= corr;
            g = g * inv_mm2;
            o[e] = valid ? g * fast_rcp(env_at(a.plan, p, T)) : 0.f;
        }
        return make_float2(o[0], o[1]);
    };

    cf* s = scratch[wave];
    const int band_lo = a.plan.band_lo, nband = a.plan.nband;
    cf w1024[NS];
#pragma unroll
    for (int r = 0; r < NS; ++r) w1024[r] = (r < 8) ? a.plan.tw1024[lane + 64 * r] : mk(-1.f, 0.f);
    float4 sc = make_float4(0.f, 0.f, 1.f, 0.f);
    float inv_bc2 = 1.f;
    int improved = 0;
    if (MODE == AN_ADJ && a.do_step) {
        sc = a.sched[min(max(*a.step - 1, 0), a.sched_len - 1)];
        inv_bc2 = 1.0f / sc.z;
        improved = a.improved[b];
    }

    const float l1g = (MODE == AN_ADJ && L1) ? a.l1_weight / (float)(nband * T) : 0.f;
    float wA[kMelTapsA], wB[kMelTapsB];
    int sA = 0, sB = 0;
    if (MELF) {
#pragma unroll
        for (int j = 0; j < kMelTapsA; ++j) wA[j] = a.melf_w[(size_t)lane * kMelTapsB + j];
#pragma unroll
        for (int j = 0; j < kMelTapsB; ++j) wB[j] = a.melf_w[(size_t)(lane + 64) * kMelTapsB + j];
        sA = a.melf_s[lane];
        sB = a.melf_s[lane + 64];
#pragma unroll
        for (int r = 0; r < 8; ++r) {
            const int f = lane + 64 * r - band_lo;
            if (f >= nband && f < kFS) magrow_s[MELF ? wave : 0][f] = 0.f;
        }
    }
    float2 raw[8];
#pragma unroll
    for (int r = 0; r < 8; ++r) raw[r] = load_half(kHop * t0 + 128 * r);

#pragma unroll 1
    for (int fr = 0; fr < nfr; ++fr) {
        const int t = t0 + fr;
        const size_t row = (size_t)(f0 + t);
        cf preP[NS];
        float preM[NS], preV[NS], preC[NS], pre0[NS];
        if (MODE == AN_ADJ) {
#pragma unroll
            for (int r = 0; r < NS; ++r) {
                const int f = lane + 64 * r - band_lo;
                const size_t idx = row * S + (size_t)min(max(f, 0), S - 1);
                preP[r] = a.phasor[idx];
                if (a.do_step) { preM[r] = a.mom[idx]; preV[r] = a.vel[idx]; preC[r] = a.coef[idx]; }
                else { preM[r] = preV[r] = 0.f; preC[r] = L1 ? a.coef[idx] : 0.f; }
                pre0[r] = (a.do_step || L1) ? a.c0[idx] : 0.f;
            }
        }
        cf v[8];
#pragma unroll
        for (int r = 0; r < 8; ++r) {
            const float2 w = wins[lane + 64 * r];
            v[r] = mk(raw[r].x * w.x, raw[r].y * w.y);
        }
#pragma unroll
        for (int r = 0; r < 6; ++r) raw[r] = raw[r + 2];
        raw[6] = load_half(kHop * (t + 1) + 768);
        raw[7] = load_half(kHop * (t + 1) + 896);
        fft512_wave_t<-1>(lane, v, tw1s, tw2s, s);

        const int src_lane = (64 - lane) & 63;
#pragma unroll
        for (int r = 0; r < NS; ++r) {
            cf zp = (r < 8) ? mk(__shfl(v[7 - r].x, src_lane), __shfl(v[7 - r].y, src_lane)) : v[0];
            if (lane == 0) zp = (r == 0 || r == 8) ? v[0] : v[8 - r];
            const int k = lane + 64 * r;
            const int f = k - band_lo;
            if (f < 0 || f >= nband || (r == 8 && lane != 0)) continue;
            const cf zk = v[r < 8 ? r : 0];
            const cf e = mk(0.5f * (zk.x + zp.x), 0.5f * (zk.y - zp.y));
            const cf d = mk(0.5f * (zk.x - zp.x), 0.5f * (zk.y + zp.y));
            const cf wd = cmul(w1024[r], d);
            const cf X = mk(e.x + wd.y, e.y - wd.x);
            const size_t idx = row * S + f;
            if (MODE == AN_NORM) {
                const float mg = fast_sqrt(X.x * X.x + X.y * X.y);
                const float im = fast_rcp(mg);
                if (MELF) magrow_s[wave][f] = mg;
                else if (a.mag) a.mag[idx] = mg;
                if (a.unit) a.unit[idx] = (mg > 0.f) ? mk(X.x * im, X.y * im) : mk(a.unit_default, 0.f);
            } else {
                const cf P = preP[r];
                float g = (X.x * P.x + X.y * P.y) * (1.0f / 512.0f);
                if (WIDE && (k == 0 || k == 512)) g = (X.x * P.x) * (1.0f / 1024.0f);
                if (L1) {
                    const float dc = preC[r] - pre0[r];
                    g += l1g * ((dc > 0.f) ? 1.f : ((dc < 0.f) ? -1.f : 0.f));
                }
                if (a.grad_out) a.grad_out[idx] = g;
                if (a.do_step) {
                    float mo = preM[r], ve = preV[r], p = preC[r];
                    float blo, bhi;
                    box_bounds(pre0[r], a.box_ratio, blo, bhi);
                    nadam_clamp_update(p, mo, ve, g, blo, bhi, sc.x, sc.y, inv_bc2, a.hyp);
                    a.mom[idx] = mo; a.vel[idx] = ve; a.coef[idx] = p;
                    if (improved) a.best[idx] = p;
                }
            }
        }
        if (MODE == AN_NORM && MELF) {
            float* mr = magrow_s[MELF ? wave : 0];
            float m0 = 0.f, m1 = 0.f;
#pragma unroll
            for (int j = 0; j < kMelTapsA; ++j) m0 += wA[j] * mr[sA + j];
#pragma unroll
            for (int j = 0; j < kMelTapsB; ++j) m1 += wB[j] * mr[sB + j];
            float* mo = a.mel_out + row * 128;
            mo[lane] = m0;
            mo[lane + 64] = m1;
        }
        if (MODE == AN_NORM && a.write_pad) {
            if (WIDE) {
                for (int f = nband + lane; f < S; f += 64) {
                    const size_t idx = row * S + f;
                    if (a.mag) a.mag[idx] = 0.f;
                    if (a.unit) a.unit[idx] = mk(0.f, 0.f);
                }
            } else {
#pragma unroll
                for (int r = 0; r < 8; ++r) {
                    const int f = lane + 64 * r - band_lo;
                    if (f >= nband && f < kFS) {
                        const size_t idx = row * kFS + f;
                        if (a.mag) a.mag[idx] = 0.f;
                        if (a.unit) a.unit[idx] = mk(0.f, 0.f);
                    }
                }
            }
        }
    }
}

template <int MODE, bool L1, bool MELG = false, bool WIDE = false>
__global__ __launch_bounds__(kSThreads, WIDE ? 3 : 4) void synth_stream_kernel(SynthArgs a) {
    static_assert(!(WIDE && MELG), "the wide layout takes the dense mel GEMM");
    constexpr int S = WIDE ? kFSWide : kFS;
    constexpr int NS = WIDE ? 9 : 8;
    __shared__ float2 melw_s[MELG ? kFS : 1];
    __shared__ float melrow_s[MELG ? kSW : 1][MELG ? 128 : 1];
    __shared__ cf tw1s[512];
    __shared__ cf tw2s[64];
    __shared__ float2 wins[512];
    __shared__ cf mcs[512];
    __shared__ cf scratch[kSW][kFftScratch];
    const int tid = threadIdx.x;
    const float scale = (MODE == SY_FWD) ? (1.0f / 512.0f) : 1.0f;
    fft_fill_tables(tid, kSThreads, a.plan.tw512, tw1s, tw2s);
    for (int i = tid; i < 512; i += kSThreads) {
        wins[i] = make_float2(a.plan.window[2 * i] * scale, a.plan.window[2 * i + 1] * scale);
        const cf w = a.plan.tw1024[i];
        mcs[i] = (WIDE || i < 256) ? mk(0.5f * (1.f + w.y), 0.5f * w.x) : mk(0.5f * (1.f - w.y), -0.5f * w.x);
    }
    if (MELG)
        for (int i = tid; i < kFS; i += kSThreads) melw_s[i] = a.melw[i];
    __syncthreads();

    int b = blockIdx.y, wgx = blockIdx.x;
    if (a.wg_tab) { const int e = a.wg_tab[blockIdx.x]; b = e >> 12; wgx = e & 4095; }
    const int f0 = a.frame_off[b];
    const int T = a.frame_off[b + 1] - f0;
    const int nblk = T - 1;
    const int wave = __builtin_amdgcn_readfirstlane(tid >> 6), lane = tid & 63;
    const int run = wgx * kSW + wave;
    int nseg, jb0, jb1;
    synth_segment(nblk, run, a.run_blocks, nseg, jb0, jb1);
    if (run >= nseg || T < 1) return;
    const bool first = jb0 == 0, last = jb1 == nblk;
    const int t_lo = max(jb0 - 1, 0);
    const int t_hi = (MODE == SY_ADJ && last) ? T + 2 : jb1 + 1;
    const int Ny = kHop * nblk;
    const int so = sig_offset(a.frame_off, b);
    float* out = a.out + so;
    const float* add = (MODE == SY_FWD && a.add) ? a.add + so : nullptr;
    const float* y = (MODE == SY_ADJ) ? a.yraw + so : nullptr;
    float inv_m = 1.f, inv_m2 = 1.f;
    if (MODE == SY_ADJ) {
        const ClipNorm cn = clip_norm_wave(a.pmax_in + (size_t)b * a.pstride, a.pcount[b], lane);
        inv_m = 1.0f / cn.m;
        inv_m2 = 1.0f / cn.m2;
// ... 159 lines not shown
                    const bool edge = (r == 0 || r == 8) && lane == 0;
                    xo[r] = mk(inA[r] * inP[r].x, edge ? 0.f : inA[r] * inP[r].y);
                    if (MODE == SY_ADJ && edge) xo[r].x *= 2.f;
                }
                const int src_lane = (64 - lane) & 63;
#pragma unroll
                for (int r = 0; r < 8; ++r) {
                    cf xp = mk(__shfl(xo[7 - r].x, src_lane), __shfl(xo[7 - r].y, src_lane));
                    if (lane == 0) xp = xo[8 - r];
                    const cf A = mcs[lane + 64 * r];
                    const cf Bm = mk(1.f - A.x, -A.y);
                    const cf xk = xo[r];
                    v[r] = mk(xk.x * A.x - xk.y * A.y + xp.x * Bm.x + xp.y * Bm.y,
                              xk.x * A.y + xk.y * A.x + xp.x * Bm.y - xp.y * Bm.x);
                }
            } else {
#pragma unroll
            for (int r = 0; r < 8; ++r) {
                const cf mc = mcs[lane + 64 * r];
                const float xr = inA[r] * inP[r].x, xi = (r < 4) ? inA[r] * inP[r].y : -(inA[r] * inP[r].y);
                v[r] = mk(xr * mc.x - xi * mc.y, xr * mc.y + xi * mc.x);
            }
            }
            load_band(min(t + 1, T - 1));
            fft512_wave_t<1>(lane, v, tw1s, tw2s, s);
#pragma unroll
            for (int r = 0; r < 8; ++r) {
                const float2 w = wins[lane + 64 * r];
                c[r] = make_float2(v[r].x * w.x, v[r].y * w.y);
            }
        }
        ola_emit(i, emit, c, e0, e1);
    }
#pragma unroll 1
    for (int t = t_fft + 1; t <= t_hi; ++t) {
        const int i = t - 2;
        const bool emit = i >= jb0 && i < jb1;
        float2 e0, e1;
        epi_operands(i, emit, e0, e1);
        float2 c[8];
#pragma unroll
        for (int r = 0; r < 8; ++r) c[r] = make_float2(0.f, 0.f);
        ola_emit(i, emit, c, e0, e1);
    }
    if (MODE == SY_FWD) {
        if (a.pmax) {
            best = wave_max64(best);
            if (lane == 0) a.pmax[(size_t)b * a.pstride + run] = best;
        }
        if (L1) {
            const double tot = wave_sum_d((double)l1);
            if (lane == 0) a.pl1[(size_t)b * a.pstride + run] = tot;
        }
    } else {
        dot = wave_sum_d(dot);
        if (lane == 0) a.pdot[(size_t)b * a.pstride + run] = dot;
    }
}

__global__ __launch_bounds__(64) void l1_reduce_kernel(const double* __restrict__ pl1, const int* __restrict__ pcount, int pstride,
                                                        const int* __restrict__ frame_off, int nband, float weight,
                                                        float* __restrict__ l1term) {
    const int b = blockIdx.x, lane = threadIdx.x;
    const double s = dot_wave(pl1 + (size_t)b * pstride, pcount[b], lane);
    const int T = frame_off[b + 1] - frame_off[b];
    if (lane == 0) l1term[b] = weight * (float)(s / (double)(nband * T));
}
void launch_l1_reduce(const double* pl1, const int* pcount, int pstride, const int* frame_off, int nband, float weight,
                      float* l1term, int B, hipStream_t st) {
    hipLaunchKernelGGL(l1_reduce_kernel, dim3(B), dim3(64), 0, st, pl1, pcount, pstride, frame_off, nband, weight, l1term);
}

bool stream_supported(const PlanDev& plan) {
    return plan.stride == kFSWide || (plan.band_lo >= 1 && plan.band_lo + plan.nband <= 257);
}

void launch_analysis_stream(const AnalysisLaunch& L, hipStream_t st) {
    AnalysisArgs a{};
    a.plan = L.plan;
    a.frame_off = L.frame_off;
    a.sig = L.sig; a.sig_off = L.sig_off; a.sig_len = L.sig_len;
    a.pmax = L.pmax; a.pcount = L.pcount; a.pstride = L.pstride;
    a.double_norm = L.double_norm; a.unit_default = L.unit_default;
    a.mag = L.mag; a.unit = (cf*)L.unit; a.full = nullptr;
    a.yraw = L.yraw; a.pdot = L.pdot; a.phasor = (const cf*)L.phasor;
    a.coef = L.coef; a.mom = L.mom; a.vel = L.vel; a.lo = L.lo; a.hi = L.hi; a.best = L.best;
    a.improved = L.improved; a.sched = (const float4*)L.sched; a.sched_len = L.sched_len > 0 ? L.sched_len : 1; a.step = L.step;
    a.grad_out = L.grad_out; a.do_step = L.do_step;
    a.hyp = make_float4(L.hyp[0], L.hyp[1], L.hyp[2], L.hyp[3]);
    a.gpad = L.gpad; a.write_pad = L.write_pad;
    a.c0 = L.c0; a.box_ratio = L.box_ratio; a.l1_weight = L.l1_weight;
    int R = 4;
    dim3 grid;
    if (L.run_frames >= 4 && L.run_frames <= 16 && L.wg_tab && L.n_wg > 0) {
        R = L.run_frames;
        a.wg_tab = L.wg_tab;
        grid = dim3((unsigned)L.n_wg, 1, 1);
    } else {
        for (int cand = 16; cand >= 4; --cand)
            if ((long)L.B * ((L.max_frames + cand - 1) / cand) >= 4096) { R = cand; break; }
        for (int cand = R; cand >= 4 && cand >= R - 3; --cand)
            if (((L.max_frames + cand - 1) / cand) % kSW == 0) { R = cand; break; }
        const int runs = (L.max_frames + R - 1) / R;
        grid = dim3((unsigned)((runs + kSW - 1) / kSW), (unsigned)L.B, 1);
    }
    if (L.plan.stride == kFSWide) {
        if (L.adjoint && a.l1_weight != 0.f) hipLaunchKernelGGL((analysis_stream_kernel<AN_ADJ, true, false, true>), grid, dim3(kSThreads), 0, st, a, R);
        else if (L.adjoint) hipLaunchKernelGGL((analysis_stream_kernel<AN_ADJ, false, false, true>), grid, dim3(kSThreads), 0, st, a, R);
        else hipLaunchKernelGGL((analysis_stream_kernel<AN_NORM, false, false, true>), grid, dim3(kSThreads), 0, st, a, R);
    } else if (L.adjoint && a.l1_weight != 0.f) hipLaunchKernelGGL((analysis_stream_kernel<AN_ADJ, true>), grid, dim3(kSThreads), 0, st, a, R);
    else if (L.adjoint) hipLaunchKernelGGL((analysis_stream_kernel<AN_ADJ, false>), grid, dim3(kSThreads), 0, st, a, R);
    else if (L.mel_out && L.melf_w && L.melf_s) {
        a.mel_out = L.mel_out; a.melf_w = L.melf_w; a.melf_s = L.melf_s; a.mag = nullptr;
        hipLaunchKernelGGL((analysis_stream_kernel<AN_NORM, false, true>), grid, dim3(kSThreads), 0, st, a, R);
    } else hipLaunchKernelGGL((analysis_stream_kernel<AN_NORM, false>), grid, dim3(kSThreads), 0, st, a, R);
}

void launch_synth_stream(const SynthLaunch& L, hipStream_t st) {
    SynthArgs a{};
    a.plan = L.plan;
    a.frame_off = L.frame_off;
    a.amp = L.amp; a.ph = (const cf*)L.ph; a.full = nullptr;
    a.out = L.out; a.add = L.add; a.pmax = L.pmax; a.pstride = L.pstride;
    a.yraw = L.yraw; a.pmax_in = L.pmax_in; a.pcount = L.pcount; a.pdot = L.pdot; a.gpad = L.gpad;
    a.c0 = L.c0; a.pl1 = (L.c0 && L.pl1) ? L.pl1 : nullptr;
    const int nblk = L.max_frames - 1;
    a.run_blocks = (L.run_blocks >= 1 && L.run_blocks <= kSynthBlocks) ? L.run_blocks : kSynthBlocks;
    int runs = (nblk + a.run_blocks - 1) / a.run_blocks;
    if (runs < 1) runs = 1;
    dim3 grid((unsigned)((runs + kSW - 1) / kSW), (unsigned)L.B, 1);
    if (L.wg_tab && L.n_wg > 0 && a.run_blocks == L.run_blocks) {
        a.wg_tab = L.wg_tab;
        grid = dim3((unsigned)L.n_wg, 1, 1);
    }
    a.dmel = L.dmel; a.melw = (const float2*)L.melw; a.melm = L.melm;
    if (L.plan.stride == kFSWide) {
        if (L.adjoint) hipLaunchKernelGGL((synth_stream_kernel<SY_ADJ, false, false, true>), grid, dim3(kSThreads), 0, st, a);
        else if (a.pl1) hipLaunchKernelGGL((synth_stream_kernel<SY_FWD, true, false, true>), grid, dim3(kSThreads), 0, st, a);
        else hipLaunchKernelGGL((synth_stream_kernel<SY_FWD, false, false, true>), grid, dim3(kSThreads), 0, st, a);
    } else if (L.adjoint && L.dmel && L.melw && L.melm) hipLaunchKernelGGL((synth_stream_kernel<SY_ADJ, false, true>), grid, dim3(kSThreads), 0, st, a);
    else if (L.adjoint) hipLaunchKernelGGL((synth_stream_kernel<SY_ADJ, false>), grid, dim3(kSThreads), 0, st, a);
    else if (a.pl1) hipLaunchKernelGGL((synth_stream_kernel<SY_FWD, true>), grid, dim3(kSThreads), 0, st, a);
    else hipLaunchKernelGGL((synth_stream_kernel<SY_FWD, false>), grid, dim3(kSThreads), 0, st, a);
}

}
```

### aware_amd/csrc/kernels.h

```cpp
#pragma once
#include <hip/hip_runtime.h>
#include <stddef.h>
#include <stdint.h>
#include "common.hpp"

namespace aware {

constexpr int kStreamWaves = 4;

struct AnalysisLaunch {
    PlanDev plan;
    const int* frame_off = nullptr;
    int B = 0, max_frames = 0;
    int run_frames = 0, n_wg = 0;
    const int* wg_tab = nullptr;
    const float* sig = nullptr;
    const int* sig_off = nullptr;
    const int* sig_len = nullptr;
    const unsigned long long* pmax = nullptr;
    const int* pcount = nullptr;
    int pstride = 0;
    int double_norm = 0;
    float unit_default = 0.f;
    float* mag = nullptr;
    void* unit = nullptr;
    void* full = nullptr;
    int adjoint = 0;
    const float* yraw = nullptr;
    const double* pdot = nullptr;
    const void* phasor = nullptr;
    float* coef = nullptr; float* mom = nullptr; float* vel = nullptr;
    const float* lo = nullptr; const float* hi = nullptr; float* best = nullptr;
    const int* improved = nullptr;
    const void* sched = nullptr;
    int sched_len = 0;
    const int* step = nullptr;
    float* grad_out = nullptr;
    int do_step = 0;
    float hyp[4] = {0.1f, 0.999f, 0.001f, 1e-8f};
    int stream = 0;
    const float* gpad = nullptr;
    int write_pad = 1;
    const float* c0 = nullptr;
    float box_ratio = 0.f;
    float l1_weight = 0.f;
    float* mel_out = nullptr;
    const float* melf_w = nullptr;
    const unsigned char* melf_s = nullptr;
};
struct SynthLaunch {
    PlanDev plan;
    const int* frame_off = nullptr;
    int B = 0, max_frames = 0;
    int n_wg = 0;
    const int* wg_tab = nullptr;
    const float* amp = nullptr;
    const void* ph = nullptr;
    const void* full = nullptr;
    float* out = nullptr;
    const float* add = nullptr;
    unsigned long long* pmax = nullptr;
    int pstride = 0;
    int adjoint = 0;
    const float* yraw = nullptr;
    const unsigned long long* pmax_in = nullptr;
    const int* pcount = nullptr;
    double* pdot = nullptr;
    int stream = 0;
    float* gpad = nullptr;
    int run_blocks = kSynthBlocks;
    const float* c0 = nullptr;
    double* pl1 = nullptr;
    const int* sig_off = nullptr;
    const int* sig_len = nullptr;
    const float* dmel = nullptr;
    const void* melw = nullptr;
    const unsigned char* melm = nullptr;
};
void launch_absmax_partials(const float* sig, const int* sig_off, const int* sig_len, unsigned long long* pmax,
                            int pstride, int B, int max_len, hipStream_t st);
void launch_analysis(const AnalysisLaunch& L, hipStream_t st);
void launch_synth(const SynthLaunch& L, hipStream_t st);
bool stream_supported(const PlanDev& plan);
void launch_analysis_stream(const AnalysisLaunch& L, hipStream_t st);
void launch_synth_stream(const SynthLaunch& L, hipStream_t st);
void launch_l1_reduce(const double* pl1, const int* pcount, int pstride, const int* frame_off, int nband, float weight,
                      float* l1term, int B, hipStream_t st);
void launch_embed_prepare(const float* c0, float* coef, float* lo, float* hi, float* mom, float* vel, float* best,
                          float* c0_keep, float ratio, size_t n, hipStream_t st);
void launch_oob_residual(const float* audio, const int* in_off, const unsigned long long* pmax, const int* pcount,
                         int pstride, const float* band, const int* frame_off, float* oob, int B, int max_frames,
                         hipStream_t st);
void launch_finish(const float* yraw, const int* frame_off, const unsigned long long* pmax, const int* pcount,
                   int pstride, const float* rescale, float* out, const int* out_off, int B, int max_frames,
                   hipStream_t st);

void launch_gemm_nt(const float* A, int lda, const float* Bt, int ldb, const float* bias, float* C, int ldc, int M,
                    int N, int K, hipStream_t st);
void launch_gemm_nt_variant(const float* A, int lda, const float* Bt, int ldb, const float* bias, float* C, int ldc,
                            int M, int N, int K, int variant, hipStream_t st);
int gemm_autotune(const float* A, int lda, const float* Bt, int ldb, float* C, int ldc, int M, int N, int K,
                  hipStream_t st);
void launch_gemm_clip(const float* A, int lda, const float* Bt, int ldb, const float* bias, float* C, int ldc, int B,
                      int nwm, int Tp, int N, int K, int epi, float* rstd_io, const float* act, hipStream_t st);
size_t x3_packed_bytes(int N, int K);
void x3_pack(const float* Wt, int N, int K, uint16_t* out);
void launch_x3_pack_dev(const float* Wt_dev, int ldw, int Nvalid, int Kvalid, int N, int K, void* out, hipStream_t st);
bool gemm_clip_x3_supported(int nwm, int N, int K, int lda);
bool mel_front_x3_supported(int T, int K, int lda);
void launch_mel_front_x3(const float* mag, int lda, const void* melTpk, const int* frame_off, const int* pool_off, float* xm,
                         float* x0, float* stats, float* gstat, int B, int T, int K, hipStream_t st, float* amax_out = nullptr);
void launch_mel_back_x3(const float* dZ, int lda, const void* wTpk, const int* frame_off, const int* pool_off, float* xm,
                        const float* stats, const float* gstat, int B, int T, int K, hipStream_t st);
void launch_gemm_clip_x3(const float* A, int lda, const void* Bpk, const float* bias, float* C, int ldc, int B, int nwm,
                         int Tp, int N, int K, int epi, float* rstd_io, const float* act, hipStream_t st,
                         const void* lastpk = nullptr, float* zpart = nullptr, int CL = 0, int Mrows = 0);
size_t h2_packed_bytes(int N, int K);
void launch_h2_pack(const float* Wt_dev, int ldw, int N, int K, void* out, hipStream_t st);
void launch_clip_amax(const float* A, int lda, int K, int rows_per_clip, int B, float* amax, hipStream_t st);
bool gemm_clip_h2_supported(int nwm, int N, int K, int lda);
void launch_gemm_clip_h2(const float* A, int lda, const void* Bpk, const float* amax_in, float* amax_out, const float* bias,
                         float* C, int ldc, int B, int nwm, int Tp, int N, int K, int epi, float* rstd_io, const float* act,
                         hipStream_t st, const void* lastpk = nullptr, float* zpart = nullptr, int CL = 0);
void launch_gemm_ragged_h2(const float* A, int lda, const void* Bpk, const float* amax_in, float* amax_out, const float* bias,
                           float* C, int ldc, int B, const int* frame_off, const int* pool_off, const int* order, int N, int K,
                           int epi, float* rstd_io, const float* act, hipStream_t st);
void launch_ragged_amax(const float* A, int lda, int K, const int* frame_off, const int* pool_off, int B, float* amax, hipStream_t st);
void launch_gemm_ragged_x3(const float* A, int lda, const void* Bpk, const float* bias, float* C, int ldc, int B,
                           const int* frame_off, const int* pool_off, const int* order, int N, int K, int epi, float* rstd_io,
                           const float* act, hipStream_t st);
bool readout_x3_supported(int nwm, int ci, int C);
void launch_readout_x3(const float* hin, int ci, const float* zpart, int nslab, const float* bias, const void* WTpk,
                       const float* rstd_prev, const float* target, float* pred, float* loss, float* best_loss, int* improved,
                       int* step, float* dZ, int B, int nwm, int Tp, int C, int nbits, int loss_kind, hipStream_t st,
                       const float* loss_add, void* img, float* amax_out = nullptr);
size_t readout_x3_image_bytes(int B, int nwm);
void launch_readout_grad_ragged_x3(const float* hin, int ci, const float* dZl, const void* WTpk, const float* rstd_prev, float* dZ,
                                   const int* frame_off, const int* pool_off, const int* order, int B, hipStream_t st,
                                   float* amax_out = nullptr);
constexpr int kMelClipFrames = 192;
void launch_mel_norm_fwd(const float* xm, const int* frame_off, const int* pool_off, float* x0, float* stats,
                         float* gstat, float* part, int pstride, int B, int max_frames, hipStream_t st,
                         float* amax_out = nullptr);
void launch_mel_norm_bwd(const float* dx0, float* xm_inout, const int* frame_off, const int* pool_off, const float* stats,
                         const float* gstat, float* part, int pstride, int B, int max_frames, hipStream_t st);
void launch_mel_norm_fwd_any(const float* xm, const int* frame_off, const int* pool_off, float* x0, float* stats, float* gstat,
                             float* part, int pstride, int B, int max_frames, int n_mels, int Mp, hipStream_t st);
void launch_mel_norm_bwd_any(const float* dx0, float* xm_inout, const int* frame_off, const int* pool_off, const float* stats,
                             const float* gstat, float* part, int pstride, int B, int max_frames, int n_mels, int Mp, hipStream_t st);
void launch_in_lrelu_fwd(float* z, const int* frame_off, const int* pool_off, float* rstd, int C, int B, int max_pooled,
                         hipStream_t st);
void launch_in_lrelu_bwd(float* dA, const float* A, const int* frame_off, const int* pool_off, const float* rstd, int C, int B,
                         int max_pooled, hipStream_t st);
constexpr int kActRelu = 0, kActLRelu = 1, kActGelu = 2, kActSwish = 3, kActTanh = 4, kActSigmoid = 5;
constexpr int kNormInstance = 0, kNormAffine = 1, kNormNone = 2;
AW_HD bool norm_act_needs_stash(int norm, int act) {
    return !(act == kActLRelu || (act == kActRelu && norm != kNormInstance));
}
void launch_norm_act_fwd(int norm, int act, float* z, const int* frame_off, const int* pool_off, float* rstd, const float* scale,
                         const float* shift, float* stash, int C, int B, int max_pooled, hipStream_t st);
void launch_norm_act_bwd(int norm, int act, float* dA, const float* A, const float* stash, const int* frame_off, const int* pool_off,
                         const float* rstd, const float* scale, int C, int B, int max_pooled, hipStream_t st);
void launch_head(const float* a3, const int* frame_off, const int* pool_off, const float* target, float* pred, float* loss,
                 float* best_loss, int* improved, float* dA3, int* step, int loss_kind, int nbits, int B,
                 hipStream_t st, const float* loss_add = nullptr, int final_act = kActTanh, int C = 0);
void launch_gemm_nt_splitk(const float* A, int lda, const float* Bt, int ldb, float* Cpart, int ldc, int M, int N, int K,
                           int ksplit, hipStream_t st);
void launch_tail(const float* zpart, int nsplit, size_t slab, const float* bias, const int* frame_off, const int* pool_off,
                 const float* target, float* pred, float* loss, float* best_loss, int* improved, float* dZ, int* step,
                 int loss_kind, int nbits, int B, int max_pooled, hipStream_t st, const float* loss_add = nullptr, int ldz = 0,
                 int C = 0);

void launch_readout_wide(const float* A, int Cp, const int* frame_off, const int* pool_off, const float* rstd, const float* target,
                         float* pred, float* loss, float* best_loss, int* improved, float* dout, float* gmax, int* step,
                         int loss_kind, int nbits, int B, hipStream_t st, const float* loss_add, int final_act, bool card_bwd);

void launch_polar_decompose(const void* spec, float* mag, float* phase, size_t n, hipStream_t st);
void launch_polar_decompose_bwd(const void* spec, const float* gmag, const float* gphase, void* gspec, size_t n, hipStream_t st);
void launch_polar_assemble(const float* mag, const float* phase, void* spec, size_t n, hipStream_t st);
void launch_polar_assemble_bwd(const float* mag, const float* phase, const void* gspec, float* gmag, float* gphase, size_t n,
                               hipStream_t st);
void launch_transpose(const float* in, float* out, int R, int C, hipStream_t st);
void launch_colsum(const float* in, float* out, int R, int C, hipStream_t st);
void launch_normalize_bwd(const float* x, const float* g, float* dx, const int* off, const int* len, int B, hipStream_t st);
void launch_nadam_clamp(float* p, const float* g, float* m, float* v, const float* lo, const float* hi, size_t n, float c_grad,
                        float c_mom, float bias_corr2, float beta1, float beta2, float eps, hipStream_t st);

void launch_opt_clamp(int kind, float* p, const float* g, float* m, float* v, const float* lo, const float* hi, size_t n,
                      const float* c4, const float* h8, hipStream_t st);
void launch_opt_rows(int kind, float* coef, const float* grad, float* mom, float* vel, const float* c0, float ratio, float* best,
                     const int* improved, const int* frame_off, int B, int NF, const double* tab, int tab_len, const int* step,
                     const double* lr_clip, double wd, const float* h8, int nband, int stride, hipStream_t st);
void launch_plateau(const float* loss, double* state, double* lr_clip, int B, double factor, int patience, double threshold,
                    double min_lr, double eps, hipStream_t st);

void launch_pcm_quantize(const float* in, float* out, const int* off, const int* len, const unsigned long long* pmax,
                         const int* pcount, int pstride, float q, float lo, float hi, int B, int max_len,
                         hipStream_t st);
void launch_normalize(const float* in, float* out, const int* off, const int* len, const unsigned long long* pmax,
                      const int* pcount, int pstride, int B, int max_len, hipStream_t st);
void launch_upfirdn(const float* in, const int* in_off, const int* in_len, float* out, const int* out_off,
                    const int* out_len, const float* h, int nh, int up, int down, int half_len, int B, int max_out,
                    hipStream_t st);
void launch_iir_full(const float* in, const int* off, const int* len, void* out, int out_f64, const double* b,
                     const double* a, const double* zi, int ncoef, int mode, double* scratch, int sstride, int B,
                     hipStream_t st);
void launch_gaussian_noise_full(const float* in, float* out, const int* off, const int* len, const unsigned* seeds,
                                double* power, float snr_db, int B, int max_len, hipStream_t st);
void launch_snr(const float* a, const int* a_off, const float* b, const int* b_off, const int* len, double* out, int B,
                hipStream_t st);
void launch_phase_vocoder(const void* in, const int* fin, void* out, const int* fout, double rate, int B, hipStream_t st);
void launch_spectral_quantize(void* spec, int nframes, float step_db, float floor_db, hipStream_t st);
void launch_spectral_quantize_bwd(const void* spec, const void* gout, void* gin, int nframes, float step_db, float floor_db,
                                  hipStream_t st);
void launch_decimate_interp(const float* in, const int* off, const int* len, double* out, int k, int B, int max_len,
                            hipStream_t st);
void launch_segment_copy(const float* in, const int* in_off, float* out, const int* out_off, const int* out_len,
                         const int* cut_start, const int* cut_len, int zero_fill, int B, int max_len, hipStream_t st);

struct GenPlanDev {
    int n_fft = 0, hop = 0, stride = 0;
    const cf* th = nullptr;
    const cf* twN = nullptr;
    const float* window = nullptr;
    const float* window2 = nullptr;
    const float* env = nullptr;
};

AW_HD float gen_env_loop(const float* w2, int N, int hop, int p, int T) {
    const int tlo = p - N + 1 > 0 ? (p - N + hop) / hop : 0;
    const int thi = (p / hop < T - 1) ? p / hop : T - 1;
    float e = 0.f;
    for (int t = tlo; t <= thi; ++t) e += w2[p - hop * t];
    return e;
}
AW_HD float gen_env(const float* env, const float* w2, int N, int hop, int p, int T) {
    if ((long)T * hop < N) return gen_env_loop(w2, N, hop, p, T);
    if (p < N) return env[p];
    const int q = p - T * hop;
    if (q >= 0) return env[N + hop + (q < N / 2 ? q : N / 2 - 1)];
    return env[N + p % hop];
}

struct GenLaunch {
    GenPlanDev plan;
    int B = 0, NF = 0, max_len = 0;
    const int* frame_off = nullptr;
    const int* sig_off = nullptr;
    const int* sig_len = nullptr;
    const int* out_off = nullptr;
    const int* out_len = nullptr;
    const unsigned long long* pmax = nullptr;
    const int* pcount = nullptr;
    int pstride = 0;
    float* frames = nullptr;
};
void launch_gen_analysis(const GenLaunch& L, const float* sig, void* spec, int adjoint, hipStream_t st);
void launch_gen_synthesis(const GenLaunch& L, const void* spec, float* out, int adjoint, hipStream_t st);
void launch_gen_normalize(const GenLaunch& L, float* out, hipStream_t st);

constexpr int kStoiFrame = 256, kStoiHop = 128, kStoiBands = 15, kStoiRow = 16, kStoiN = 30;
constexpr int kStoiSegChunk = 64;
AW_HD int stoi_frames(int n) { return n > kStoiFrame ? (n - kStoiFrame + kStoiHop - 1) / kStoiHop : 0; }
AW_HD int stoi_partials(int n) {
    const int nseg = stoi_frames(n) - 1 - (kStoiN - 1);
    return nseg > 0 ? (nseg + kStoiSegChunk - 1) / kStoiSegChunk : 1;
}
struct StoiTables {
    const cf* th = nullptr;
    const cf* twN = nullptr;
    const float* window = nullptr;
    const int* bands = nullptr;
};
struct StoiLaunch {
    StoiTables tab;
// ... 118 lines not shown
```

### aware_amd/csrc/seam_kernels.hip

```cpp
#include "common.hpp"
#include "dsp_args.hpp"
#include "kernels.h"

namespace aware {

__global__ __launch_bounds__(256) void polar_decompose_kernel(const cf* __restrict__ spec, float* __restrict__ mag,
                                                              float* __restrict__ phase, size_t n) {
    for (size_t i = (size_t)blockIdx.x * 256 + threadIdx.x; i < n; i += (size_t)gridDim.x * 256) {
        const cf s = spec[i];
        mag[i] = hypotf(s.x, s.y);
        if (phase) phase[i] = atan2f(s.y, s.x);
    }
}
__global__ __launch_bounds__(256) void polar_decompose_bwd_kernel(const cf* __restrict__ spec, const float* __restrict__ gmag,
                                                                  const float* __restrict__ gphase, cf* __restrict__ gspec, size_t n) {
    for (size_t i = (size_t)blockIdx.x * 256 + threadIdx.x; i < n; i += (size_t)gridDim.x * 256) {
        const cf s = spec[i];
        const float r = hypotf(s.x, s.y);
        cf g = mk(0.f, 0.f);
        if (r > 0.f) {
            const float ir = 1.0f / r;
            if (gmag) { const float gm = gmag[i]; g.x += gm * s.x * ir; g.y += gm * s.y * ir; }
            if (gphase) { const float gp = gphase[i] * ir * ir; g.x += -gp * s.y; g.y += gp * s.x; }
        }
// ... 9 lines not shown
        spec[i] = mk(m * cs, m * sn);
    }
}
__global__ __launch_bounds__(256) void polar_assemble_bwd_kernel(const float* __restrict__ mag, const float* __restrict__ phase,
                                                                 const cf* __restrict__ gspec, float* __restrict__ gmag,
                                                                 float* __restrict__ gphase, size_t n) {
    for (size_t i = (size_t)blockIdx.x * 256 + threadIdx.x; i < n; i += (size_t)gridDim.x * 256) {
        float sn, cs;
        sincosf(phase[i], &sn, &cs);
        const cf g = gspec[i];
        if (gmag) gmag[i] = g.x * cs + g.y * sn;
        if (gphase) gphase[i] = mag[i] * (g.y * cs - g.x * sn);
    }
}

__global__ __launch_bounds__(256) void normalize_bwd_kernel(const float* __restrict__ x, const float* __restrict__ g,
                                                            float* __restrict__ dx, const int* __restrict__ off,
                                                            const int* __restrict__ len) {
    __shared__ unsigned long long red[4];
    __shared__ double dred[4];
    const int b = blockIdx.x, tid = threadIdx.x;
    const int n = len[b];
    const float* xb = x + off[b];
    const float* gb = g + off[b];
    float* db = dx + off[b];
    unsigned long long v = 0;
    double s = 0.0;
    for (int i = tid; i < n; i += 256) {
        const float xv = xb[i];
        v = umax64(v, pack_max(fabsf(xv), (unsigned)i));
        s += (double)gb[i] * (double)xv;
    }
    v = wave_max64(v);
    s = wave_sum_d(s);
    if ((tid & 63) == 0) { red[tid >> 6] = v; dred[tid >> 6] = s; }
    __syncthreads();
    v = umax64(umax64(red[0], red[1]), umax64(red[2], red[3]));
    const double dot = (dred[0] + dred[1]) + (dred[2] + dred[3]);
    const float m = __uint_as_float((unsigned)(v >> 32)) + 1e-8f;
    const unsigned k = 0xFFFFFFFFu - (unsigned)(v & 0xFFFFFFFFu);
    const float xk = n > 0 ? xb[min(k, (unsigned)(n - 1))] : 0.f;
    const float sk = (xk > 0.f) ? 1.f : ((xk < 0.f) ? -1.f : 0.f);
    const float corr = sk * (float)(dot / ((double)m * (double)m));
    for (int i = tid; i < n; i += 256) {
        float d = gb[i] / m;
        if ((unsigned)i == k) d -= corr;
        db[i] = d;
    }
}

__global__ __launch_bounds__(256) void nadam_clamp_kernel(float* __restrict__ p, const float* __restrict__ g,
                                                          float* __restrict__ m, float* __restrict__ v,
                                                          const float* __restrict__ lo, const float* __restrict__ hi, size_t n,
                                                          float c_grad, float c_mom, float inv_bc2, float4 hyp) {
    for (size_t i = (size_t)blockIdx.x * 256 + threadIdx.x; i < n; i += (size_t)gridDim.x * 256) {
        float mo = m[i], ve = v[i], pv = p[i];
        nadam_clamp_update(pv, mo, ve, g[i], lo ? lo[i] : -INFINITY, hi ? hi[i] : INFINITY, c_grad, c_mom, inv_bc2, hyp);
        m[i] = mo; v[i] = ve; p[i] = pv;
    }
}

__global__ __launch_bounds__(256) void opt_clamp_kernel(int kind, float* __restrict__ p, const float* __restrict__ g,
                                                        float* __restrict__ m, float* __restrict__ v,
                                                        const float* __restrict__ lo, const float* __restrict__ hi, size_t n,
                                                        float4 c, OptHyp H) {
    for (size_t i = (size_t)blockIdx.x * 256 + threadIdx.x; i < n; i += (size_t)gridDim.x * 256) {
        float mo = m[i], ve = v[i], pv = p[i];
        opt_clamp_update(kind, pv, mo, ve, g[i], lo ? lo[i] : -INFINITY, hi ? hi[i] : INFINITY, c, H);
        m[i] = mo; v[i] = ve; p[i] = pv;
    }
}
void launch_opt_clamp(int kind, float* p, const float* g, float* m, float* v, const float* lo, const float* hi, size_t n,
                      const float* c4, const float* h8, hipStream_t st) {
    OptHyp H;
    for (int i = 0; i < 8; ++i) H.h[i] = h8[i];
    const size_t blocks = (n + 255) / 256;
    hipLaunchKernelGGL(opt_clamp_kernel, dim3((unsigned)(blocks > 4096 ? 4096 : blocks)), dim3(256), 0, st, kind, p, g, m, v, lo, hi,
                       n, make_float4(c4[0], c4[1], c4[2], c4[3]), H);
}

__global__ __launch_bounds__(256) void opt_rows_kernel(int kind, float* __restrict__ coef, const float* __restrict__ grad,
                                                       float* __restrict__ mom, float* __restrict__ vel,
                                                       const float* __restrict__ c0, float ratio, float* __restrict__ best,
                                                       const int* __restrict__ improved, const int* __restrict__ frame_off, int B,
                                                       const double* __restrict__ tab, int tab_len, const int* __restrict__ step,
                                                       const double* __restrict__ lr_clip, double wd, OptHyp H, int nband,
                                                       int stride) {
    const int row = blockIdx.x;
    int lo_ = 0, hi_ = B;
    while (hi_ - lo_ > 1) {
        const int mid = (lo_ + hi_) >> 1;
        if (frame_off[mid] <= row) lo_ = mid; else hi_ = mid;
    }
    const int clip = lo_;
    if ((int)threadIdx.x >= nband) return;
    const int t = min(max(*step - 1, 0), tab_len - 1);
    const double* e = tab + (size_t)t * 5;
    const double lr = lr_clip ? lr_clip[clip] : e[3];
    if (e[4] >= 0.0) H.h[0] = (float)e[4];
    float4 c;
    c.x = (float)(lr * e[0]);
    c.y = kind == OPT_SGD ? (float)e[1] : (float)(lr * e[1]);
    c.z = (float)e[2];
    c.w = (float)(1.0 - lr * wd);
    for (int f = threadIdx.x; f < nband; f += blockDim.x) {
        const size_t idx = (size_t)row * stride + f;
        float p = coef[idx], mo = mom[idx], ve = vel[idx], blo, bhi;
        box_bounds(c0[idx], ratio, blo, bhi);
        opt_clamp_update(kind, p, mo, ve, grad[idx], blo, bhi, c, H);
        coef[idx] = p; mom[idx] = mo; vel[idx] = ve;
        if (improved[clip]) best[idx] = p;
    }
}
void launch_opt_rows(int kind, float* coef, const float* grad, float* mom, float* vel, const float* c0, float ratio, float* best,
                     const int* improved, const int* frame_off, int B, int NF, const double* tab, int tab_len, const int* step,
                     const double* lr_clip, double wd, const float* h8, int nband, int stride, hipStream_t st) {
    OptHyp H;
    for (int i = 0; i < 8; ++i) H.h[i] = h8[i];
    hipLaunchKernelGGL(opt_rows_kernel, dim3(NF), dim3(256), 0, st, kind, coef, grad, mom, vel, c0, ratio, best, improved, frame_off,
                       B, tab, tab_len, step, lr_clip, wd, H, nband, stride);
}

__global__ __launch_bounds__(256) void plateau_kernel(const float* __restrict__ loss, double* __restrict__ state,
                                                      double* __restrict__ lr_clip, int B, double factor, int patience,
                                                      double threshold, double min_lr, double eps) {
    const int b = blockIdx.x * 256 + threadIdx.x;
    if (b >= B) return;
    const double cur = (double)loss[b];
    double best = state[3 * b], bad = state[3 * b + 1];
    if (cur < best * (1.0 - threshold)) { best = cur; bad = 0.0; }
    else bad += 1.0;
    if (bad > (double)patience) {
        const double old = lr_clip[b], nw = fmax(old * factor, min_lr);
        if (old - nw > eps) lr_clip[b] = nw;
        bad = 0.0;
    }
    state[3 * b] = best; state[3 * b + 1] = bad;
}
void launch_plateau(const float* loss, double* state, double* lr_clip, int B, double factor, int patience, double threshold,
                    double min_lr, double eps, hipStream_t st) {
    hipLaunchKernelGGL(plateau_kernel, dim3((B + 255) / 256), dim3(256), 0, st, loss, state, lr_clip, B, factor, patience, threshold,
                       min_lr, eps);
}

__global__ __launch_bounds__(256) void transpose_kernel(const float* __restrict__ in, float* __restrict__ out, int R, int C) {
    __shared__ float tile[32][33];
    const int c0 = blockIdx.x * 32, r0 = blockIdx.y * 32;
    const int tx = threadIdx.x & 31, ty = threadIdx.x >> 5;
    for (int i = ty; i < 32; i += 8) {
        const int r = r0 + i, c = c0 + tx;
        tile[i][tx] = (r < R && c < C) ? in[(size_t)r * C + c] : 0.f;
    }
    __syncthreads();
    for (int i = ty; i < 32; i += 8) {
        const int c = c0 + i, r = r0 + tx;
        if (c < C && r < R) out[(size_t)c * R + r] = tile[tx][i];
    }
}
__global__ __launch_bounds__(256) void colsum_kernel(const float* __restrict__ in, float* __restrict__ out, int R, int C) {
    __shared__ double red[8][32];
    const int c = blockIdx.x * 32 + (threadIdx.x & 31), g = threadIdx.x >> 5;
    double s = 0.0;
    if (c < C)
        for (int r = g; r < R; r += 8) s += (double)in[(size_t)r * C + c];
    red[g][threadIdx.x & 31] = s;
    __syncthreads();
    if (g == 0 && c < C) {
        double t = 0.0;
        for (int i = 0; i < 8; ++i) t += red[i][threadIdx.x & 31];
        out[c] = (float)t;
    }
}
void launch_transpose(const float* in, float* out, int R, int C, hipStream_t st) {
    hipLaunchKernelGGL(transpose_kernel, dim3((C + 31) / 32, (R + 31) / 32), dim3(256), 0, st, in, out, R, C);
}
void launch_colsum(const float* in, float* out, int R, int C, hipStream_t st) {
    hipLaunchKernelGGL(colsum_kernel, dim3((C + 31) / 32), dim3(256), 0, st, in, out, R, C);
}

static inline unsigned gridn(size_t n) {
    size_t g = (n + 255) / 256;
    return (unsigned)(g < 1 ? 1 : (g > 16384 ? 16384 : g));
}
void launch_polar_decompose(const void* spec, float* mag, float* phase, size_t n, hipStream_t st) {
    hipLaunchKernelGGL(polar_decompose_kernel, dim3(gridn(n)), dim3(256), 0, st, (const cf*)spec, mag, phase, n);
}
void launch_polar_decompose_bwd(const void* spec, const float* gmag, const float* gphase, void* gspec, size_t n, hipStream_t st) {
    hipLaunchKernelGGL(polar_decompose_bwd_kernel, dim3(gridn(n)), dim3(256), 0, st, (const cf*)spec, gmag, gphase, (cf*)gspec, n);
}
void launch_polar_assemble(const float* mag, const float* phase, void* spec, size_t n, hipStream_t st) {
    hipLaunchKernelGGL(polar_assemble_kernel, dim3(gridn(n)), dim3(256), 0, st, mag, phase, (cf*)spec, n);
}
void launch_polar_assemble_bwd(const float* mag, const float* phase, const void* gspec, float* gmag, float* gphase, size_t n,
                               hipStream_t st) {
    hipLaunchKernelGGL(polar_assemble_bwd_kernel, dim3(gridn(n)), dim3(256), 0, st, mag, phase, (const cf*)gspec, gmag, gphase, n);
}
void launch_normalize_bwd(const float* x, const float* g, float* dx, const int* off, const int* len, int B, hipStream_t st) {
    hipLaunchKernelGGL(normalize_bwd_kernel, dim3(B), dim3(256), 0, st, x, g, dx, off, len);
}
void launch_nadam_clamp(float* p, const float* g, float* m, float* v, const float* lo, const float* hi, size_t n, float c_grad,
                        float c_mom, float bias_corr2, float beta1, float beta2, float eps, hipStream_t st) {
    const float4 hyp = make_float4(1.0f - beta1, beta2, 1.0f - beta2, eps);
    hipLaunchKernelGGL(nadam_clamp_kernel, dim3(gridn(n)), dim3(256), 0, st, p, g, m, v, lo, hi, n, c_grad, c_mom,
// ... 5 lines not shown
```

### aware_amd/runtime.py

```python
from __future__ import annotations

import ctypes as C
from typing import Sequence

import numpy as np
import torch

from . import _lib
from ._lib import AwareHipError, DetectorArch, EmbedConfig, check, load_library, require_gpu

SPEC_STRIDE = 256
SPEC_STRIDE_WIDE = 576
FULL_STRIDE = 520
CONV_PIPES = {"f16x2": 0, "f32": 1, "bf16x3": 2}
LOSS_KINDS = {"push_extremes": 0, "mse": 1, "hinge": 2, "sign": 3, "push_sigmoid": 4, "ber": 5, "push_extremes_l1": 6}


def band_stride(band_lo: int, band_hi: int) -> int:
    return SPEC_STRIDE if band_lo >= 1 and band_hi <= 511 and band_hi - band_lo + 1 <= SPEC_STRIDE else SPEC_STRIDE_WIDE


def stored_channels(channels: Sequence[int]) -> list[int]:
    n = len(channels) - 1
    out = []
# ... 126 lines not shown
        self.out_lengths = [self.lib.aware_batch_out_length(h, i) for i in range(self.B)]
        self.frame_offsets = np.concatenate([[0], np.cumsum(self.frames)]).tolist()
        self.total_in = self.in_offsets[-1] + self.lengths[-1]
        self.scratch_bytes = self.lib.aware_batch_scratch_bytes(h)
        self.uniform = len(set(self.lengths)) == 1 and in_offsets is None

    def __del__(self):
        try:
            if getattr(self, "h", None):
                self.lib.aware_batch_destroy(self.h)
                self.h = None
        except Exception:
            pass

    def scratch(self):
        return torch.empty(self.scratch_bytes, dtype=torch.uint8, device=_dev())

    def pack(self, clips) -> torch.Tensor:
        out = torch.zeros(self.total_in, dtype=torch.float32, device=_dev())
        for c, o, n in zip(clips, self.in_offsets, self.lengths):
            out[o:o + n] = torch.as_tensor(c, dtype=torch.float32)
        return out

    def unpack_out(self, flat: torch.Tensor):
        return [flat[o:o + n] for o, n in zip(self.out_offsets, self.out_lengths)]


def stft(plan: Plan, batch: Batch, audio: torch.Tensor, normalize=False) -> torch.Tensor:
    spec = torch.empty((batch.total_frames, plan.spectrum_stride), dtype=torch.complex64, device=audio.device)
    scr = batch.scratch()
    check(plan.lib.aware_stft(plan.h, batch.h, _ptr(audio), int(normalize), _ptr(spec), _ptr(scr), _stream()), "aware_stft")
    return spec


def istft(plan: Plan, batch: Batch, spec: torch.Tensor, normalize=False) -> torch.Tensor:
    out = torch.empty(batch.total_out, dtype=torch.float32, device=spec.device)
    scr = batch.scratch()
    rc = plan.lib.aware_istft(plan.h, batch.h, _ptr(spec), int(normalize), _ptr(out), _ptr(scr), _stream())
    _check_nola(rc, plan, batch)
    check(rc, "aware_istft")
    return out


def _check_nola(rc: int, plan: Plan, batch: Batch):
    if rc == -1 and plan.general and batch.plan is plan:
        bad = [n for n in batch.lengths if not nola_ok(plan.n_fft, plan.hop, plan.win_length, plan.window, n)]
        if bad:
            raise RuntimeError(f"istft: window overlap-add envelope is below 1e-11 (NOLA condition violated) for n_fft "
                               f"{plan.n_fft}, hop {plan.hop}, win_length {plan.win_length}, {plan.window} window; torch.istft "
                               f"raises for this geometry too")


def stft_band(plan: Plan, batch: Batch, audio: torch.Tensor, normalize=True):
    mag = torch.empty((batch.total_frames, plan.band_stride), dtype=torch.float32, device=audio.device)
    ph = torch.empty((batch.total_frames, plan.band_stride), dtype=torch.complex64, device=audio.device)
    scr = batch.scratch()
    check(plan.lib.aware_stft_band(plan.h, batch.h, _ptr(audio), int(normalize), _ptr(mag), _ptr(ph), _ptr(scr), _stream()),
          "aware_stft_band")
    return mag, ph


def stft_bwd(plan: Plan, batch: Batch, grad_spec: torch.Tensor) -> torch.Tensor:
    out = torch.zeros(batch.total_in, dtype=torch.float32, device=grad_spec.device)
    check(plan.lib.aware_stft_bwd(plan.h, batch.h, _ptr(grad_spec), _ptr(out), _stream()), "aware_stft_bwd")
    return out


def istft_bwd(plan: Plan, batch: Batch, grad_audio: torch.Tensor) -> torch.Tensor:
    gs = torch.empty((batch.total_frames, plan.spectrum_stride), dtype=torch.complex64, device=grad_audio.device)
    rc = plan.lib.aware_istft_bwd(plan.h, batch.h, _ptr(grad_audio), _ptr(gs), _stream())
    _check_nola(rc, plan, batch)
    check(rc, "aware_istft_bwd")
    return gs


def polar_decompose(spec: torch.Tensor):
    lib = load_library()
    mag = torch.empty(spec.shape, dtype=torch.float32, device=spec.device)
    ph = torch.empty(spec.shape, dtype=torch.float32, device=spec.device)
    check(lib.aware_polar_decompose(_ptr(spec), _ptr(mag), _ptr(ph), spec.numel(), _stream()), "aware_polar_decompose")
    return mag, ph


def polar_decompose_bwd(spec, grad_mag, grad_phase):
    lib = load_library()
    gs = torch.empty_like(spec)
    check(lib.aware_polar_decompose_bwd(_ptr(spec), _ptr(grad_mag), _ptr(grad_phase), _ptr(gs), spec.numel(), _stream()),
          "aware_polar_decompose_bwd")
    return gs


def polar_assemble(mag: torch.Tensor, phase: torch.Tensor) -> torch.Tensor:
    lib = load_library()
    spec = torch.empty(mag.shape, dtype=torch.complex64, device=mag.device)
    check(lib.aware_polar_assemble(_ptr(mag), _ptr(phase), _ptr(spec), mag.numel(), _stream()), "aware_polar_assemble")
    return spec


def polar_assemble_bwd(mag, phase, grad_spec, need_mag=True, need_phase=True):
    lib = load_library()
    gm = torch.empty_like(mag) if need_mag else None
    gp = torch.empty_like(mag) if need_phase else None
    check(lib.aware_polar_assemble_bwd(_ptr(mag), _ptr(phase), _ptr(grad_spec), _ptr(gm), _ptr(gp), mag.numel(), _stream()),
          "aware_polar_assemble_bwd")
    return gm, gp


def waveform_normalize_bwd(x: "Ragged", grad_out: torch.Tensor) -> torch.Tensor:
    lib = load_library()
    gi = torch.empty_like(x.data)
    check(lib.aware_waveform_normalize_bwd(_ptr(x.data), _ptr(grad_out), _ptr(gi), _ptr(x.d_off), _ptr(x.d_len), x.B, _stream()),
          "aware_waveform_normalize_bwd")
    return gi


class OptClamp:

    def __init__(self, param: torch.Tensor, name: str, num_steps: int, scheduler_name: str | None = None, scheduler_params=None,
                 **params):
        from .embedding.optimizers import get_optimizer, hyper_parameters, step_table
        from .embedding.schedulers import get_scheduler
        self.lib = load_library()
        self.param = param
        self.opt = get_optimizer(name, None, **params)
        sched = get_scheduler(scheduler_name, self.opt, num_steps, **(scheduler_params or {})) if scheduler_name else None
        if sched is not None and sched["plateau"] is not None:
            raise NotImplementedError("OptClamp: a firing ReduceLROnPlateau needs the per-clip state of an embed session")
        self.hyp = hyper_parameters(self.opt)
        self.table = step_table(self.opt, num_steps, sched["torch"] if sched else None)
        self.s1 = torch.zeros_like(param)
        self.s2 = torch.zeros_like(param)
        self.t = 0

    def step(self, grad: torch.Tensor, lo: torch.Tensor | None = None, hi: torch.Tensor | None = None):
        from .embedding.optimizers import step_scalars
        self.t += 1
        c4, h8 = step_scalars(self.opt, self.table, self.t, hyp=self.hyp)
        check(self.lib.aware_opt_clamp_step(self.opt["kind"], _ptr(self.param), _ptr(grad), _ptr(self.s1), _ptr(self.s2), _ptr(lo),
                                            _ptr(hi), self.param.numel(), c4.ctypes.data_as(C.POINTER(C.c_float)),
                                            h8.ctypes.data_as(C.POINTER(C.c_float)), _stream()), "aware_opt_clamp_step")


class NAdamClamp:

    def __init__(self, param: torch.Tensor, lr=0.1, betas=(0.9, 0.999), eps=1e-8, momentum_decay=4e-3):
        self.lib = load_library()
        self.param = param
        self.lr, self.betas, self.eps, self.md = float(lr), (float(betas[0]), float(betas[1])), float(eps), float(momentum_decay)
        self.exp_avg = torch.zeros_like(param)
        self.exp_avg_sq = torch.zeros_like(param)
        self.mu_product = C.c_float(1.0)
        self.t = 0

    def step(self, grad: torch.Tensor, lo: torch.Tensor | None = None, hi: torch.Tensor | None = None):
        self.t += 1
        c3 = (C.c_float * 3)()
        check(self.lib.aware_nadam_coefficients(self.t, self.lr, self.betas[0], self.betas[1], self.md, C.byref(self.mu_product), c3),
              "aware_nadam_coefficients")
        check(self.lib.aware_nadam_clamp_step(_ptr(self.param), _ptr(grad), _ptr(self.exp_avg), _ptr(self.exp_avg_sq), _ptr(lo),
                                              _ptr(hi), self.param.numel(), c3, self.betas[0], self.betas[1], self.eps, _stream()),
              "aware_nadam_clamp_step")


def detector_backward(plan: Plan, det: "DetectorWeights", batch: Batch, mag: torch.Tensor, grad_values: torch.Tensor):
    nbytes = plan.lib.aware_detector_backward_workspace_bytes(batch.h, det.h)
    ws = torch.empty(nbytes, dtype=torch.uint8, device=mag.device)
# ... 197 lines not shown
        else:
            ent = la.device_entries(chain, sample_rate)
            arr = (_lib.LoopAttack * len(ent))(*[_lib.LoopAttack(k, p, pr) for k, p, pr in ent])
            nbytes = self.lib.aware_embed_loop_attack_workspace_bytes(self.batch.h, len(ent))
            ws = torch.empty(nbytes, dtype=torch.uint8, device=_dev())
            rc = self.lib.aware_embed_set_loop_attacks(self.h, arr, len(ent), sd, _ptr(ws), nbytes, _stream())
        if rc == -1:
            raise ValueError("set_loop_attacks: refused (it has to precede the first iterate(); see aware_hip.h)")
        check(rc, "aware_embed_set_loop_attacks")
        self.loop_attacks, self._la_ws = chain, ws

    @property
    def attacked(self):
        p = self.lib.aware_embed_buffer(self.h, 12)
        if not p:
            return None
        off = p - self._la_ws.data_ptr()
        return self._la_ws[off: off + 4 * self.batch.total_out].view(torch.float32)

    @property
    def impulse_responses(self):
        p = self.lib.aware_embed_buffer(self.h, 13)
        if not p:
            return None
        off = p - self._la_ws.data_ptr()
        return self._la_ws[off: off + 4 * 8192 * self.batch.B].view(torch.float32).view(self.batch.B, 8192)

    def begin(self, audio: torch.Tensor, target: torch.Tensor):
        self._audio, self._target = audio, target.contiguous().float()
        check(self.lib.aware_embed_begin(self.h, _ptr(audio), _ptr(self._target), _stream()), "aware_embed_begin")

    def iterate(self, n: int):
        rc = self.lib.aware_embed_iterate(self.h, int(n), _stream())
        if rc == -1:
            raise ValueError(f"iterate({n}): more than num_iterations = {self.cfg.num_iterations} steps since begin()")
        check(rc, "aware_embed_iterate")

    def gradient(self) -> torch.Tensor:
        g = torch.zeros((self.batch.total_frames, self.plan.band_stride), dtype=torch.float32, device=self.ws.device)
        check(self.lib.aware_embed_gradient(self.h, _ptr(g), _stream()), "aware_embed_gradient")
        return g

    def finish(self, rescale: torch.Tensor | None = None) -> torch.Tensor:
        out = torch.empty(self.batch.total_out, dtype=torch.float32, device=self.ws.device)
        check(self.lib.aware_embed_finish(self.h, _ptr(rescale), _ptr(out), _stream()), "aware_embed_finish")
        return out

    def _view(self, which, shape, dtype=torch.float32):
        p = self.lib.aware_embed_buffer(self.h, which)
        n = int(np.prod(shape))
        off = p - self.ws.data_ptr()
        itemsize = torch.empty((), dtype=dtype).element_size()
        return self.ws[off: off + n * itemsize].view(dtype).view(*shape)

    @property
    def loss(self):
        return self._view(0, (self.batch.B,))

    @property
    def best_loss(self):
        return self._view(1, (self.batch.B,))

    @property
    def pred(self):
        return self._view(2, (self.batch.B, self.det.n_bits))

    @property
    def coef(self):
        return self._view(3, (self.batch.total_frames, self.plan.band_stride))

    @property
    def best_coef(self):
        return self._view(4, (self.batch.total_frames, self.plan.band_stride))

    @property
    def bounds(self):
        return (self._view(5, (self.batch.total_frames, self.plan.band_stride)),
                self._view(6, (self.batch.total_frames, self.plan.band_stride)))

    @property
    def step(self):
        return self._view(8, (1,), torch.int32)

    def clip_learning_rates(self) -> np.ndarray:
        if not self.lib.aware_embed_buffer(self.h, 11):
            raise AwareHipError("no optimiser was set with set_optimizer")
        return self._view(11, (self.batch.B,), torch.float64).cpu().numpy()


def gemm_nt(a: torch.Tensor, bt: torch.Tensor, bias: torch.Tensor | None = None) -> torch.Tensor:
    lib = load_library()
    M, K = a.shape
    N = bt.shape[0]
    c = torch.empty((M, N), dtype=torch.float32, device=a.device)
    check(lib.aware_gemm_nt(_ptr(a), a.stride(0), _ptr(bt), bt.stride(0), _ptr(bias), _ptr(c), N, M, N, K, _stream()),
          "aware_gemm_nt")
    return c


def x3_pack(wt: torch.Tensor) -> torch.Tensor:
    lib = load_library()
    w = np.ascontiguousarray(wt.detach().cpu().numpy(), dtype=np.float32)
    N, K = w.shape
    nbytes = int(lib.aware_x3_packed_bytes(N, K))
    if nbytes == 0:
        raise AwareHipError("aware_x3_pack: N must be a positive multiple of 16")
    out = np.zeros(nbytes, dtype=np.uint8)
    check(lib.aware_x3_pack(w.ctypes.data, N, K, out.ctypes.data), "aware_x3_pack")
    return torch.from_numpy(out).cuda()


def gemm_clip(a: torch.Tensor, bt: torch.Tensor, bias, B: int, Tp: int, epi: int = 0, rstd=None, act=None,
              mode: int = 0, packed=None):
    lib = load_library()
    M, K = a.shape
    N = bt.shape[0]
    c = torch.empty((M, N), dtype=torch.float32, device=a.device)
    if rstd is None:
        rstd = torch.zeros((B, N), dtype=torch.float32, device=a.device)
    if mode == 1 and packed is None:
        packed = x3_pack(bt)
    check(lib.aware_gemm_clip(_ptr(a), a.stride(0), _ptr(bt), bt.stride(0), _ptr(packed), _ptr(bias), _ptr(c), N, B, Tp, N, K,
                              epi, _ptr(rstd), _ptr(act), mode, _stream()), "aware_gemm_clip")
    return c, rstd


def gemm_clip_h2(a: torch.Tensor, bt: torch.Tensor, bias, B: int, Tp: int, epi: int = 0, rstd=None, act=None, w_last=None):
    lib = load_library()
    M, K = a.shape
    N = bt.shape[0]
    dev = a.device
    btd = bt.to(dev).contiguous()
    c = torch.empty((M, N), dtype=torch.float32, device=dev)
    if rstd is None:
        rstd = torch.zeros((B, N), dtype=torch.float32, device=dev)
    amax = torch.zeros((B, 64), dtype=torch.float32, device=dev)
    nbytes = int(lib.aware_gemm_clip_h2_workspace_bytes(B, N, K))
    ws = torch.empty(nbytes, dtype=torch.uint8, device=dev)
    pkl, zpart, CL = None, None, 0
    if w_last is not None:
        CL = w_last.shape[0]
        wl = torch.zeros((16 * ((CL + 15) // 16), N), dtype=torch.float32)
        wl[:CL] = w_last.detach().cpu().float()
        pkl = x3_pack(wl)
        zpart = torch.zeros((N // 128, M, CL), dtype=torch.float32, device=dev)
    check(lib.aware_gemm_clip_h2(_ptr(a), a.stride(0), _ptr(btd), btd.stride(0), _ptr(bias), _ptr(c), N, B, Tp, N, K, epi, _ptr(rstd),
                                 _ptr(act), _ptr(pkl), _ptr(zpart), CL, _ptr(amax), _ptr(ws), nbytes, _stream()), "aware_gemm_clip_h2")
    torch.cuda.current_stream().synchronize()
    return (c, rstd, amax) if w_last is None else (c, rstd, amax, zpart)


def gemm_clip_last(a: torch.Tensor, bt: torch.Tensor, bias, w_last: torch.Tensor, B: int, Tp: int):
    lib = load_library()
    M, K = a.shape
    N = bt.shape[0]
    CL = w_last.shape[0]
    clp = 16 * ((CL + 15) // 16)
    wl = torch.zeros((clp, N), dtype=torch.float32)
    wl[:CL] = w_last.detach().cpu().float()
    c = torch.empty((M, N), dtype=torch.float32, device=a.device)
    rstd = torch.zeros((B, N), dtype=torch.float32, device=a.device)
    zpart = torch.zeros((N // 128, M, CL), dtype=torch.float32, device=a.device)
    pk, pkl = x3_pack(bt), x3_pack(wl)
    check(lib.aware_gemm_clip_last(_ptr(a), a.stride(0), _ptr(pk), _ptr(bias), _ptr(c), N, B, Tp, N, K, _ptr(rstd),
                                   _ptr(pkl), _ptr(zpart), CL, _stream()), "aware_gemm_clip_last")
    torch.cuda.current_stream().synchronize()
# ... 350 lines not shown
```

### include/aware_hip.h

```cpp
#ifndef AWARE_HIP_H
#define AWARE_HIP_H

#include <stddef.h>
#include <stdint.h>

#ifdef __cplusplus
extern "C" {
#endif

#define AWARE_OK 0
#define AWARE_E_BADARG (-1)
#define AWARE_E_UNSUPPORTED (-2)
#define AWARE_E_HIP (-3)
#define AWARE_E_WORKSPACE (-4)

#define AWARE_LOSS_PUSH_EXTREMES 0
#define AWARE_LOSS_MSE 1
#define AWARE_LOSS_HINGE 2
#define AWARE_LOSS_SIGN 3
#define AWARE_LOSS_PUSH_SIGMOID 4
#define AWARE_LOSS_BER 5
#define AWARE_LOSS_PUSH_L1 6
#define AWARE_LOSS_EXTERNAL 7

#define AWARE_SPEC_STRIDE 256
#define AWARE_SPEC_STRIDE_WIDE 576
#define AWARE_FULL_STRIDE 520

typedef struct aware_plan aware_plan;
typedef struct aware_detector aware_detector;
typedef struct aware_batch aware_batch;
typedef struct aware_embed aware_embed;
typedef struct aware_stoi_plan aware_stoi_plan;

int aware_version(void);
const char* aware_last_hip_error(void);

int aware_plan_create(aware_plan** out, int n_fft, int hop, int win_length, int window,
                      int band_lo_bin, int band_hi_bin);
void aware_plan_destroy(aware_plan* plan);
#define AWARE_PLAN_GENERAL 1
int aware_plan_create_ex(aware_plan** out, int n_fft, int hop, int win_length, int window, int band_lo_bin,
                         int band_hi_bin, int flags);
int aware_plan_spectrum_stride(const aware_plan* plan);
int aware_plan_is_general(const aware_plan* plan);
int aware_plan_band_stride(const aware_plan* plan);
int aware_nola_check(int n_fft, int hop, int win_length, int window, int n_samples);

int aware_batch_create(aware_batch** out, int B, const int* n_samples, const int* in_offsets);
void aware_batch_destroy(aware_batch* batch);
int aware_batch_total_frames(const aware_batch* batch);
int aware_batch_total_pooled(const aware_batch* batch);
int aware_batch_total_out(const aware_batch* batch);
int aware_batch_out_offset(const aware_batch* batch, int b);
int aware_batch_out_length(const aware_batch* batch, int b);
int aware_batch_frames(const aware_batch* batch, int b);
int aware_batch_create_for_plan(aware_batch** out, const aware_plan* plan, int B, const int* n_samples,
                                const int* in_offsets);

size_t aware_batch_scratch_bytes(const aware_batch* batch);
int aware_stft(const aware_plan* plan, const aware_batch* batch, const float* audio, int normalize,
               void* spec, void* scratch, void* stream);
int aware_istft(const aware_plan* plan, const aware_batch* batch, const void* spec, int normalize,
                float* out, void* scratch, void* stream);
int aware_stft_band(const aware_plan* plan, const aware_batch* batch, const float* audio, int normalize,
                    float* mag, void* phasor, void* scratch, void* stream);

int aware_stft_bwd(const aware_plan* plan, const aware_batch* batch, const void* grad_spec, float* grad_audio,
                   void* stream);
int aware_istft_bwd(const aware_plan* plan, const aware_batch* batch, const float* grad_audio, void* grad_spec,
                    void* stream);

int aware_polar_decompose(const void* spec, float* mag, float* phase, size_t n, void* stream);
int aware_polar_decompose_bwd(const void* spec, const float* grad_mag, const float* grad_phase, void* grad_spec, size_t n,
                              void* stream);
int aware_polar_assemble(const float* mag, const float* phase, void* spec, size_t n, void* stream);
int aware_polar_assemble_bwd(const float* mag, const float* phase, const void* grad_spec, float* grad_mag,
                             float* grad_phase, size_t n, void* stream);
int aware_waveform_normalize_bwd(const float* in, const float* grad_out, float* grad_in, const int* off, const int* len,
                                 int B, void* stream);
int aware_nadam_coefficients(int step, float lr, float beta1, float beta2, float momentum_decay, float* mu_product_io,
                             float* coef3);
int aware_nadam_clamp_step(float* param, const float* grad, float* exp_avg, float* exp_avg_sq, const float* lo,
                           const float* hi, size_t n, const float* coef3, float beta1, float beta2, float eps, void* stream);

int aware_detector_create(aware_detector** out, const aware_plan* plan, const float* mel_basis, int n_mels,
                          int n_layers, const int* channels, const float* const* weights,
                          const float* const* biases);
void aware_detector_destroy(aware_detector* det);

#define AWARE_ACT_RELU 0
#define AWARE_ACT_LEAKY_RELU 1
#define AWARE_ACT_GELU 2
#define AWARE_ACT_SWISH 3
#define AWARE_NORM_INSTANCE 0
#define AWARE_NORM_BATCH 1
#define AWARE_NORM_NONE 2
#define AWARE_FINAL_RELU 0
#define AWARE_FINAL_LEAKY_RELU 1
#define AWARE_FINAL_GELU 2
#define AWARE_FINAL_SWISH 3
#define AWARE_FINAL_TANH 4
#define AWARE_FINAL_SIGMOID 5
typedef struct aware_detector_arch {
    int activation;
    int norm;
    int final_activation;
    const float* const* norm_scale;
    const float* const* norm_shift;
} aware_detector_arch;
int aware_detector_create_ex(aware_detector** out, const aware_plan* plan, const float* mel_basis, int n_mels,
                             int n_layers, const int* channels, const float* const* weights,
                             const float* const* biases, const aware_detector_arch* arch);
int aware_detector_is_card(const aware_detector* det);

size_t aware_detect_workspace_bytes(const aware_batch* batch, const aware_detector* det);
int aware_detect(const aware_plan* plan, const aware_detector* det, const aware_batch* batch,
                 const float* audio, float* values, void* workspace, size_t workspace_bytes, void* stream);
int aware_detector_forward(const aware_detector* det, const aware_batch* batch, const float* mag,
                           float* values, void* workspace, size_t workspace_bytes, void* stream);

size_t aware_detector_backward_workspace_bytes(const aware_batch* batch, const aware_detector* det);
int aware_detector_backward(const aware_detector* det, const aware_batch* batch, const float* mag,
                            const float* grad_values, float* values, float* grad_mag, void* workspace,
                            size_t workspace_bytes, void* stream);

size_t aware_detector_train_workspace_bytes(const aware_batch* batch, const aware_detector* det);
int aware_detector_weight_gradients(const aware_detector* det, const aware_batch* batch, const float* mag,
                                    const float* grad_values, float* values, float* grad_mag,
                                    float* const* grad_weights, float* const* grad_biases, void* workspace,
                                    size_t workspace_bytes, void* stream);
int aware_detector_update(aware_detector* det, const float* mel_basis, const float* const* weights,
                          const float* const* biases);
int aware_detector_train_gradients(const aware_detector* det, const aware_batch* batch, const float* mag, const float* target,
                                   int loss_kind, float* loss_out, float* values, float* grad_mag,
                                   float* const* grad_weights, float* const* grad_biases, void* workspace,
                                   size_t workspace_bytes, void* stream);
int aware_detector_update_device(aware_detector* det, const float* const* dev_weights, const float* const* dev_biases,
                                 void* stream);

typedef struct aware_embed_config {
    int num_iterations;
    float tolerance_db;
    int loss;
    float lr, beta1, beta2, eps, momentum_decay;
    int use_graph;
    int conv_pipe;
    int readout;
    int dsp_path;
    float l1_weight;
    int mel;
} aware_embed_config;

#define AWARE_OPT_NADAM 0
#define AWARE_OPT_ADAM 1
#define AWARE_OPT_ADAMW 2
// ... 113 lines not shown
```

Measured before the change: 1952.

## Recompute phasor and c0 from stored spectrum; defer best-snapshot writes by one step

```diff
diff --git a/aware_amd/_lib.py b/aware_amd/_lib.py
--- a/aware_amd/_lib.py
+++ b/aware_amd/_lib.py
@@ -105,6 +105,7 @@
     "aware_detector_backward_workspace_bytes": (_sz, [_vp, _vp]),
     "aware_detector_backward": (_i, [_vp, _vp, _vp, _vp, _vp, _vp, _vp, _sz, _vp]),
     "aware_polar_decompose": (_i, [_vp, _vp, _vp, _sz, _vp]),
+    "aware_polar_split": (_i, [_vp, _vp, _vp, _sz, _f, _vp]),
     "aware_polar_decompose_bwd": (_i, [_vp, _vp, _vp, _vp, _sz, _vp]),
     "aware_polar_assemble": (_i, [_vp, _vp, _vp, _sz, _vp]),
     "aware_polar_assemble_bwd": (_i, [_vp, _vp, _vp, _vp, _vp, _sz, _vp]),
diff --git a/aware_amd/csrc/capi.hip b/aware_amd/csrc/capi.hip
--- a/aware_amd/csrc/capi.hip
+++ b/aware_amd/csrc/capi.hip
@@ -1494,6 +1494,8 @@
     return AWARE_OK;
 }
 
+static constexpr float kUnitDefault0 = 1.f;
+
 struct aware_embed {
     const aware_plan* plan;
     const aware_detector* det;
@@ -1502,6 +1504,8 @@
     DetBufs db;
     float *coef, *lo, *hi, *mom, *vel, *best, *mag, *gmag;
     cf *P, *U;
+    cf* X0 = nullptr;
+    int* best_live = nullptr;
     float *yraw, *oob, *gy;
     float* gpad;
     float* c0 = nullptr;
@@ -1573,6 +1577,8 @@
     e->pmaxY = c.take<unsigned long long>((size_t)b->B * b->pstride);
     e->pdot = c.take<double>((size_t)b->B * b->pstride);
     e->c0 = c.take<float>(nsp);
+    e->X0 = c.take<cf>(nsp);
+    e->best_live = c.take<int>((size_t)b->B * 2);
     e->opt.d_tab = c.take<double>((size_t)iters * 5);
     e->opt.d_lr = c.take<double>(b->B);
     e->opt.d_state = c.take<double>((size_t)b->B * 3);
@@ -1631,6 +1637,12 @@
 extern "C" int aware_polar_decompose(const void* spec, float* mag, float* phase, size_t n, void* stream) {
     if (!spec || !mag || n < 1) return AWARE_E_BADARG;
     launch_polar_decompose(spec, mag, phase, n, (hipStream_t)stream);
+    LAUNCHCHK();
+    return AWARE_OK;
+}
+extern "C" int aware_polar_split(const void* spec, float* mag, void* unit, size_t n, float unit_default, void* stream) {
+    if (!spec || !mag || !unit || n < 1) return AWARE_E_BADARG;
+    launch_polar_split(spec, mag, unit, n, unit_default, (hipStream_t)stream);
     LAUNCHCHK();
     return AWARE_OK;
 }
@@ -1975,6 +1987,9 @@
         case 11: return e->opt.active ? e->opt.d_lr : nullptr;
         case 12: return e->la.n ? e->la.z : nullptr;
         case 13: return (e->la.n && e->la.rv >= 0) ? e->la.h : nullptr;
+        case 14: return e->X0;
+        case 15: return e->mom;
+        case 16: return e->vel;
         default: return nullptr;
     }
 }
@@ -1989,7 +2004,7 @@
     L.plan = e->plan->dev; L.frame_off = b->d_frame_off; L.B = b->B; L.max_frames = b->max_frames; L.run_frames = b->an_run; L.wg_tab = b->d_an_wg; L.n_wg = b->n_an_wg;
     L.sig = audio; L.sig_off = b->d_in_off; L.sig_len = b->d_in_len;
     L.pmax = e->pmaxA; L.pcount = b->d_pc_in; L.pstride = b->pstride;
-    L.mag = e->mag; L.unit = e->P; L.unit_default = 1.f;
+    L.mag = e->mag; L.unit = e->P; L.unit_default = kUnitDefault0; L.x0 = e->X0;
     run_analysis(L, e->cfg.dsp_path, st);
     LAUNCHCHK();
     SynthLaunch S;
@@ -2005,6 +2020,7 @@
     LAUNCHCHK();
     HIPCHK(hipMemcpyAsync(e->target, target, (size_t)b->B * e->det->nbits * sizeof(float), hipMemcpyDeviceToDevice, st));
     HIPCHK(hipMemsetAsync(e->step, 0, 4 * sizeof(int), st));
+    HIPCHK(hipMemsetAsync(e->best_live, 0, (size_t)b->B * 2 * sizeof(int), st));
     HIPCHK(hipMemsetD32Async((hipDeviceptr_t)e->best_loss, 0x7F800000, b->B, st));
     if (e->opt.active) {
         HIPCHK(hipMemcpyAsync(e->opt.d_lr, e->opt.lr_init.data(), (size_t)b->B * sizeof(double), hipMemcpyHostToDevice, st));
@@ -2039,6 +2055,15 @@
     C.h = la.h; C.h_stride = kReverbMaxIr; C.nh = la.nh; C.parts = kReverbParts; C.adjoint = adjoint; C.skip_h = adjoint;
     C.hspec = la.hspec; C.xspec = la.xspec;
     return C;
+}
+
+static int embed_flush_best(aware_embed* e, hipStream_t st) {
+    const aware_batch* b = e->b;
+    launch_best_flush(e->coef, e->best, e->best_live, b->d_frame_off, b->B, b->NF, e->step, e->plan->dev.nband,
+                      e->plan->dev.stride, st);
+    LAUNCHCHK();
+    HIPCHK(hipMemsetAsync(e->best_live, 0, (size_t)b->B * 2 * sizeof(int), st));
+    return AWARE_OK;
 }
 
 static int embed_iteration(aware_embed* e, hipStream_t st, int do_step, float* grad_out) {
@@ -2146,20 +2171,21 @@
     LA.plan = e->plan->dev; LA.frame_off = b->d_frame_off; LA.B = b->B; LA.max_frames = b->max_frames; LA.run_frames = b->an_run; LA.wg_tab = b->d_an_wg; LA.n_wg = b->n_an_wg;
     LA.sig = e->gy; LA.sig_off = b->d_out_off; LA.sig_len = b->d_out_len;
     LA.pmax = e->pmaxY; LA.pcount = b->d_pc_syn; LA.pstride = b->pstride;
-    LA.adjoint = 1; LA.yraw = e->yraw; LA.pdot = e->pdot; LA.phasor = e->P;
+    LA.adjoint = 1; LA.yraw = e->yraw; LA.pdot = e->pdot; LA.phasor = e->P; LA.x0 = e->X0; LA.unit_default = kUnitDefault0;
     LA.coef = e->coef; LA.mom = e->mom; LA.vel = e->vel; LA.lo = e->lo; LA.hi = e->hi; LA.best = e->best;
+    LA.best_live = e->best_live;
     LA.improved = e->improved; LA.sched = e->sched; LA.sched_len = e->cfg.num_iterations + 1; LA.step = e->step;
     const bool own_step = do_step && e->opt.active;
     LA.grad_out = own_step ? e->gmag : grad_out; LA.do_step = own_step ? 0 : do_step;
     memcpy(LA.hyp, e->hyp, sizeof(LA.hyp));
-    LA.gpad = e->gpad; LA.c0 = e->c0; LA.box_ratio = (float)pow(10.0, -(double)e->cfg.tolerance_db / 20.0);
+    LA.gpad = e->gpad; LA.box_ratio = (float)pow(10.0, -(double)e->cfg.tolerance_db / 20.0);
     LA.l1_weight = e->pl1 ? e->cfg.l1_weight : 0.f;
     if (attacked) { LA.pdot = e->la.pdot; LA.gpad = e->la.gpad0; }
     run_analysis(LA, dsp, st);
     LAUNCHCHK(); PROF(K_ANALYSIS_ADJ);
     if (own_step) {
         const auto& o = e->opt;
-        launch_opt_rows(o.kind, e->coef, e->gmag, e->mom, e->vel, e->c0, LA.box_ratio, e->best, e->improved, b->d_frame_off, b->B,
+        launch_opt_rows(o.kind, e->coef, e->gmag, e->mom, e->vel, e->c0, LA.box_ratio, e->best, e->best_live, e->improved, b->d_frame_off, b->B,
                         b->NF, o.d_tab, e->cfg.num_iterations, e->step, o.plateau ? o.d_lr : nullptr, o.wd, o.hyp,
                         e->plan->dev.nband, e->plan->dev.stride, st);
         if (o.plateau)
@@ -2180,7 +2206,7 @@
             if (rc) return rc;
             ++e->steps_done;
         }
-        return AWARE_OK;
+        return n_iters > 0 ? embed_flush_best(e, st) : AWARE_OK;
     }
     constexpr int kGraphIters = 16;
     if (!e->gexec) {
@@ -2207,7 +2233,7 @@
     int left = n_iters;
     for (; left >= kGraphIters; left -= kGraphIters) { HIPCHK(hipGraphLaunch(e->gexecN, st)); e->steps_done += kGraphIters; }
     for (; left > 0; --left) { HIPCHK(hipGraphLaunch(e->gexec, st)); ++e->steps_done; }
-    return AWARE_OK;
+    return n_iters > 0 ? embed_flush_best(e, st) : AWARE_OK;
 }
 
 extern "C" int aware_embed_profile(aware_embed* e, int n_iters, int max_entries, float* ms_out, int* kind_out,
@@ -2222,6 +2248,7 @@
     int rc = AWARE_OK;
     for (int i = 0; i < n_iters && rc == AWARE_OK; ++i) { rc = embed_iteration(e, st, 1, nullptr); if (rc == AWARE_OK) ++e->steps_done; }
     g_prof = nullptr;
+    if (rc == AWARE_OK) rc = embed_flush_best(e, st);
     hipError_t se = hipStreamSynchronize(st);
     int n = 0;
     for (size_t i = 1; i < p.ev.size(); ++i) {
diff --git a/aware_amd/csrc/dsp_args.hpp b/aware_amd/csrc/dsp_args.hpp
--- a/aware_amd/csrc/dsp_args.hpp
+++ b/aware_amd/csrc/dsp_args.hpp
@@ -78,6 +78,26 @@
     hi = __fadd_rn(c0, d);
 }
 
+__device__ __forceinline__ void polar_split(cf X, float unit_default, float& mg, cf& unit) {
+    mg = fast_sqrt(__fmaf_rn(X.x, X.x, __fmul_rn(X.y, X.y)));
+    const float im = fast_rcp(mg);
+    unit = (mg > 0.f) ? mk(__fmul_rn(X.x, im), __fmul_rn(X.y, im)) : mk(unit_default, 0.f);
+}
+
+struct BestRule {
+    bool save_old;
+    bool save_new;
+};
+__device__ __forceinline__ BestRule best_rule(int* live, int b, int step, int improved, bool writer) {
+    BestRule r;
+    if (!live) { r.save_old = false; r.save_new = improved != 0; return r; }
+    const int par = step & 1;
+    r.save_old = !improved && live[2 * b + par] != 0;
+    r.save_new = false;
+    if (writer) live[2 * b + (par ^ 1)] = improved;
+    return r;
+}
+
 enum { AN_NORM = 0, AN_ADJ = 1 };
 enum { SY_FWD = 0, SY_ADJ = 1 };
 
@@ -96,6 +116,7 @@
     float* mag;
     cf* unit;
     cf* full;
+    cf* x0;
     const float* yraw;
     const double* pdot;
     const cf* phasor;
@@ -105,6 +126,7 @@
     const float* lo;
     const float* hi;
     float* best;
+    int* best_live;
     const int* improved;
     const float4* sched;
     int sched_len;
@@ -114,7 +136,6 @@
     float4 hyp;
     const float* gpad;
     int write_pad;
-    const float* c0;
     float box_ratio;
     float l1_weight;
     float* mel_out;
diff --git a/aware_amd/csrc/dsp_kernels.hip b/aware_amd/csrc/dsp_kernels.hip
--- a/aware_amd/csrc/dsp_kernels.hip
+++ b/aware_amd/csrc/dsp_kernels.hip
@@ -120,11 +120,13 @@
     const int S = a.plan.stride;
     float4 sc = make_float4(0.f, 0.f, 1.f, 0.f);
     float inv_bc2 = 1.f;
-    int improved = 0;
+    BestRule br;
+    br.save_old = br.save_new = false;
     if (MODE == AN_ADJ && a.do_step) {
-        sc = a.sched[min(max(*a.step - 1, 0), a.sched_len - 1)];
+        const int step = *a.step;
+        sc = a.sched[min(max(step - 1, 0), a.sched_len - 1)];
         inv_bc2 = 1.0f / sc.z;
-        improved = a.improved[b];
+        br = best_rule(a.best_live, b, step, a.improved[b], t0 == 0 && tid == 0);
     }
 
     const bool pre_ok = (MODE == AN_ADJ) && a.do_step && band_lo < 64;
@@ -185,10 +187,12 @@
                 }
                 cf X = (r < 8) ? rfft_split_bin(k, v[r < 8 ? r : 0], s, a.plan.tw1024) : mk(rfft_split_nyquist(s), 0.f);
                 if (MODE == AN_NORM) {
-                    const float mg = fast_sqrt(X.x * X.x + X.y * X.y);
-                    const float im = fast_rcp(mg);
+                    float mg;
+                    cf un;
+                    polar_split(X, a.unit_default, mg, un);
                     if (a.mag) a.mag[idx] = mg;
-                    if (a.unit) a.unit[idx] = (mg > 0.f) ? mk(X.x * im, X.y * im) : mk(a.unit_default, 0.f);
+                    if (a.unit) a.unit[idx] = un;
+                    if (a.x0) a.x0[idx] = X;
                 } else {
                     const bool pre = pre_ok && r < 5;
                     cf P = pre ? preP[r < 5 ? r : 0] : a.phasor[idx];
@@ -200,9 +204,10 @@
                         if (pre) { mo = preM[r < 5 ? r : 0]; ve = preV[r < 5 ? r : 0]; p = preC[r < 5 ? r : 0];
                                    blo = preL[r < 5 ? r : 0]; bhi = preH[r < 5 ? r : 0]; }
                         else { mo = a.mom[idx]; ve = a.vel[idx]; p = a.coef[idx]; blo = a.lo[idx]; bhi = a.hi[idx]; }
+                        if (br.save_old) a.best[idx] = p;
                         nadam_clamp_update(p, mo, ve, g, blo, bhi, sc.x, sc.y, inv_bc2, a.hyp);
                         a.mom[idx] = mo; a.vel[idx] = ve; a.coef[idx] = p;
-                        if (improved) a.best[idx] = p;
+                        if (br.save_new) a.best[idx] = p;
                     }
                 }
             }
@@ -469,9 +474,9 @@
     a.sig = L.sig; a.sig_off = L.sig_off; a.sig_len = L.sig_len;
     a.pmax = L.pmax; a.pcount = L.pcount; a.pstride = L.pstride;
     a.double_norm = L.double_norm; a.unit_default = L.unit_default;
-    a.mag = L.mag; a.unit = (cf*)L.unit; a.full = (cf*)L.full;
+    a.mag = L.mag; a.unit = (cf*)L.unit; a.full = (cf*)L.full; a.x0 = L.adjoint ? nullptr : (cf*)L.x0;
     a.yraw = L.yraw; a.pdot = L.pdot; a.phasor = (const cf*)L.phasor;
-    a.coef = L.coef; a.mom = L.mom; a.vel = L.vel; a.lo = L.lo; a.hi = L.hi; a.best = L.best;
+    a.coef = L.coef; a.mom = L.mom; a.vel = L.vel; a.lo = L.lo; a.hi = L.hi; a.best = L.best; a.best_live = L.best_live;
     a.improved = L.improved; a.sched = (const float4*)L.sched; a.sched_len = L.sched_len > 0 ? L.sched_len : 1; a.step = L.step;
     a.grad_out = L.grad_out; a.do_step = L.do_step;
     a.hyp = make_float4(L.hyp[0], L.hyp[1], L.hyp[2], L.hyp[3]);
diff --git a/aware_amd/csrc/dsp_stream.hip b/aware_amd/csrc/dsp_stream.hip
--- a/aware_amd/csrc/dsp_stream.hip
+++ b/aware_amd/csrc/dsp_stream.hip
@@ -146,11 +146,13 @@
     for (int r = 0; r < NS; ++r) w1024[r] = (r < 8) ? a.plan.tw1024[lane + 64 * r] : mk(-1.f, 0.f);
     float4 sc = make_float4(0.f, 0.f, 1.f, 0.f);
     float inv_bc2 = 1.f;
-    int improved = 0;
+    BestRule br;
+    br.save_old = br.save_new = false;
     if (MODE == AN_ADJ && a.do_step) {
-        sc = a.sched[min(max(*a.step - 1, 0), a.sched_len - 1)];
+        const int step = *a.step;
+        sc = a.sched[min(max(step - 1, 0), a.sched_len - 1)];
         inv_bc2 = 1.0f / sc.z;
-        improved = a.improved[b];
+        br = best_rule(a.best_live, b, step, a.improved[b], t0 == 0 && lane == 0);
     }
 
     const float l1g = (MODE == AN_ADJ && L1) ? a.l1_weight / (float)(nband * T) : 0.f;
@@ -177,17 +179,16 @@
     for (int fr = 0; fr < nfr; ++fr) {
         const int t = t0 + fr;
         const size_t row = (size_t)(f0 + t);
-        cf preP[NS];
-        float preM[NS], preV[NS], preC[NS], pre0[NS];
+        cf preX[NS];
+        float preM[NS], preV[NS], preC[NS];
         if (MODE == AN_ADJ) {
 #pragma unroll
             for (int r = 0; r < NS; ++r) {
                 const int f = lane + 64 * r - band_lo;
                 const size_t idx = row * S + (size_t)min(max(f, 0), S - 1);
-                preP[r] = a.phasor[idx];
+                preX[r] = a.x0[idx];
                 if (a.do_step) { preM[r] = a.mom[idx]; preV[r] = a.vel[idx]; preC[r] = a.coef[idx]; }
                 else { preM[r] = preV[r] = 0.f; preC[r] = L1 ? a.coef[idx] : 0.f; }
-                pre0[r] = (a.do_step || L1) ? a.c0[idx] : 0.f;
             }
         }
         cf v[8];
@@ -217,27 +218,32 @@
             const cf X = mk(e.x + wd.y, e.y - wd.x);
             const size_t idx = row * S + f;
             if (MODE == AN_NORM) {
-                const float mg = fast_sqrt(X.x * X.x + X.y * X.y);
-                const float im = fast_rcp(mg);
+                float mg;
+                cf un;
+                polar_split(X, a.unit_default, mg, un);
                 if (MELF) magrow_s[wave][f] = mg;
                 else if (a.mag) a.mag[idx] = mg;
-                if (a.unit) a.unit[idx] = (mg > 0.f) ? mk(X.x * im, X.y * im) : mk(a.unit_default, 0.f);
+                if (a.unit) a.unit[idx] = un;
+                if (!MELF && a.x0) a.x0[idx] = X;
             } else {
-                const cf P = preP[r];
+                float c0;
+                cf P;
+                polar_split(preX[r], a.unit_default, c0, P);
                 float g = (X.x * P.x + X.y * P.y) * (1.0f / 512.0f);
                 if (WIDE && (k == 0 || k == 512)) g = (X.x * P.x) * (1.0f / 1024.0f);
                 if (L1) {
-                    const float dc = preC[r] - pre0[r];
+                    const float dc = preC[r] - c0;
                     g += l1g * ((dc > 0.f) ? 1.f : ((dc < 0.f) ? -1.f : 0.f));
                 }
                 if (a.grad_out) a.grad_out[idx] = g;
                 if (a.do_step) {
                     float mo = preM[r], ve = preV[r], p = preC[r];
                     float blo, bhi;
-                    box_bounds(pre0[r], a.box_ratio, blo, bhi);
+                    box_bounds(c0, a.box_ratio, blo, bhi);
                     nadam_clamp_update(p, mo, ve, g, blo, bhi, sc.x, sc.y, inv_bc2, a.hyp);
                     a.mom[idx] = mo; a.vel[idx] = ve; a.coef[idx] = p;
-                    if (improved) a.best[idx] = p;
+                    if (br.save_old) a.best[idx] = preC[r];
+                    if (br.save_new) a.best[idx] = p;
                 }
             }
         }
@@ -563,14 +569,14 @@
     a.sig = L.sig; a.sig_off = L.sig_off; a.sig_len = L.sig_len;
     a.pmax = L.pmax; a.pcount = L.pcount; a.pstride = L.pstride;
     a.double_norm = L.double_norm; a.unit_default = L.unit_default;
-    a.mag = L.mag; a.unit = (cf*)L.unit; a.full = nullptr;
+    a.mag = L.mag; a.unit = (cf*)L.unit; a.full = nullptr; a.x0 = (cf*)L.x0;
     a.yraw = L.yraw; a.pdot = L.pdot; a.phasor = (const cf*)L.phasor;
-    a.coef = L.coef; a.mom = L.mom; a.vel = L.vel; a.lo = L.lo; a.hi = L.hi; a.best = L.best;
+    a.coef = L.coef; a.mom = L.mom; a.vel = L.vel; a.lo = L.lo; a.hi = L.hi; a.best = L.best; a.best_live = L.best_live;
     a.improved = L.improved; a.sched = (const float4*)L.sched; a.sched_len = L.sched_len > 0 ? L.sched_len : 1; a.step = L.step;
     a.grad_out = L.grad_out; a.do_step = L.do_step;
     a.hyp = make_float4(L.hyp[0], L.hyp[1], L.hyp[2], L.hyp[3]);
     a.gpad = L.gpad; a.write_pad = L.write_pad;
-    a.c0 = L.c0; a.box_ratio = L.box_ratio; a.l1_weight = L.l1_weight;
+    a.box_ratio = L.box_ratio; a.l1_weight = L.l1_weight;
     int R = 4;
     dim3 grid;
     if (L.run_frames >= 4 && L.run_frames <= 16 && L.wg_tab && L.n_wg > 0) {
diff --git a/aware_amd/csrc/kernels.h b/aware_amd/csrc/kernels.h
--- a/aware_amd/csrc/kernels.h
+++ b/aware_amd/csrc/kernels.h
@@ -25,12 +25,14 @@
     float* mag = nullptr;
     void* unit = nullptr;
     void* full = nullptr;
+    void* x0 = nullptr;
     int adjoint = 0;
     const float* yraw = nullptr;
     const double* pdot = nullptr;
     const void* phasor = nullptr;
     float* coef = nullptr; float* mom = nullptr; float* vel = nullptr;
     const float* lo = nullptr; const float* hi = nullptr; float* best = nullptr;
+    int* best_live = nullptr;
     const int* improved = nullptr;
     const void* sched = nullptr;
     int sched_len = 0;
@@ -41,7 +43,6 @@
     int stream = 0;
     const float* gpad = nullptr;
     int write_pad = 1;
-    const float* c0 = nullptr;
     float box_ratio = 0.f;
     float l1_weight = 0.f;
     float* mel_out = nullptr;
@@ -189,8 +190,11 @@
 void launch_opt_clamp(int kind, float* p, const float* g, float* m, float* v, const float* lo, const float* hi, size_t n,
                       const float* c4, const float* h8, hipStream_t st);
 void launch_opt_rows(int kind, float* coef, const float* grad, float* mom, float* vel, const float* c0, float ratio, float* best,
-                     const int* improved, const int* frame_off, int B, int NF, const double* tab, int tab_len, const int* step,
+                     int* best_live, const int* improved, const int* frame_off, int B, int NF, const double* tab, int tab_len, const int* step,
                      const double* lr_clip, double wd, const float* h8, int nband, int stride, hipStream_t st);
+void launch_best_flush(const float* coef, float* best, const int* best_live, const int* frame_off, int B, int NF, const int* step,
+                       int nband, int stride, hipStream_t st);
+void launch_polar_split(const void* x, float* mag, void* unit, size_t n, float unit_default, hipStream_t st);
 void launch_plateau(const float* loss, double* state, double* lr_clip, int B, double factor, int patience, double threshold,
                     double min_lr, double eps, hipStream_t st);
 
diff --git a/aware_amd/csrc/seam_kernels.hip b/aware_amd/csrc/seam_kernels.hip
--- a/aware_amd/csrc/seam_kernels.hip
+++ b/aware_amd/csrc/seam_kernels.hip
@@ -115,7 +115,7 @@
 __global__ __launch_bounds__(256) void opt_rows_kernel(int kind, float* __restrict__ coef, const float* __restrict__ grad,
                                                        float* __restrict__ mom, float* __restrict__ vel,
                                                        const float* __restrict__ c0, float ratio, float* __restrict__ best,
-                                                       const int* __restrict__ improved, const int* __restrict__ frame_off, int B,
+                                                       int* __restrict__ best_live, const int* __restrict__ improved, const int* __restrict__ frame_off, int B,
                                                        const double* __restrict__ tab, int tab_len, const int* __restrict__ step,
                                                        const double* __restrict__ lr_clip, double wd, OptHyp H, int nband,
                                                        int stride) {
@@ -127,7 +127,9 @@
     }
     const int clip = lo_;
     if ((int)threadIdx.x >= nband) return;
-    const int t = min(max(*step - 1, 0), tab_len - 1);
+    const int s = *step;
+    const int t = min(max(s - 1, 0), tab_len - 1);
+    const BestRule br = best_rule(best_live, clip, s, improved[clip], row == frame_off[clip] && threadIdx.x == 0);
     const double* e = tab + (size_t)t * 5;
     const double lr = lr_clip ? lr_clip[clip] : e[3];
     if (e[4] >= 0.0) H.h[0] = (float)e[4];
@@ -139,19 +141,56 @@
     for (int f = threadIdx.x; f < nband; f += blockDim.x) {
         const size_t idx = (size_t)row * stride + f;
         float p = coef[idx], mo = mom[idx], ve = vel[idx], blo, bhi;
+        if (br.save_old) best[idx] = p;
         box_bounds(c0[idx], ratio, blo, bhi);
         opt_clamp_update(kind, p, mo, ve, grad[idx], blo, bhi, c, H);
         coef[idx] = p; mom[idx] = mo; vel[idx] = ve;
-        if (improved[clip]) best[idx] = p;
-    }
+        if (br.save_new) best[idx] = p;
+    }
+}
+
+__global__ __launch_bounds__(256) void best_flush_kernel(const float* __restrict__ coef, float* __restrict__ best,
+                                                         const int* __restrict__ best_live, const int* __restrict__ frame_off,
+                                                         int B, const int* __restrict__ step, int nband, int stride) {
+    const int row = blockIdx.x;
+    int lo_ = 0, hi_ = B;
+    while (hi_ - lo_ > 1) {
+        const int mid = (lo_ + hi_) >> 1;
+        if (frame_off[mid] <= row) lo_ = mid; else hi_ = mid;
+    }
+    if (!best_live[2 * lo_ + ((*step & 1) ^ 1)]) return;
+    for (int f = threadIdx.x; f < nband; f += blockDim.x) {
+        const size_t idx = (size_t)row * stride + f;
+        best[idx] = coef[idx];
+    }
+}
+void launch_best_flush(const float* coef, float* best, const int* best_live, const int* frame_off, int B, int NF, const int* step,
+                       int nband, int stride, hipStream_t st) {
+    hipLaunchKernelGGL(best_flush_kernel, dim3(NF), dim3(256), 0, st, coef, best, best_live, frame_off, B, step, nband, stride);
+}
+
+__global__ __launch_bounds__(256) void polar_split_kernel(const cf* __restrict__ x, float* __restrict__ mag, cf* __restrict__ unit,
+                                                          size_t n, float unit_default) {
+    for (size_t i = (size_t)blockIdx.x * blockDim.x + threadIdx.x; i < n; i += (size_t)gridDim.x * blockDim.x) {
+        float mg;
+        cf un;
+        polar_split(x[i], unit_default, mg, un);
+        mag[i] = mg;
+        unit[i] = un;
+    }
+}
+void launch_polar_split(const void* x, float* mag, void* unit, size_t n, float unit_default, hipStream_t st) {
+    const size_t blocks = (n + 255) / 256;
+    hipLaunchKernelGGL(polar_split_kernel, dim3((unsigned)(blocks > 4096 ? 4096 : blocks)), dim3(256), 0, st, (const cf*)x, mag,
+                       (cf*)unit, n, unit_default);
 }
 void launch_opt_rows(int kind, float* coef, const float* grad, float* mom, float* vel, const float* c0, float ratio, float* best,
-                     const int* improved, const int* frame_off, int B, int NF, const double* tab, int tab_len, const int* step,
+                     int* best_live, const int* improved, const int* frame_off, int B, int NF, const double* tab, int tab_len, const int* step,
                      const double* lr_clip, double wd, const float* h8, int nband, int stride, hipStream_t st) {
     OptHyp H;
     for (int i = 0; i < 8; ++i) H.h[i] = h8[i];
-    hipLaunchKernelGGL(opt_rows_kernel, dim3(NF), dim3(256), 0, st, kind, coef, grad, mom, vel, c0, ratio, best, improved, frame_off,
-                       B, tab, tab_len, step, lr_clip, wd, H, nband, stride);
+    hipLaunchKernelGGL(opt_rows_kernel, dim3(NF), dim3(256), 0, st, kind, coef, grad, mom, vel, c0, ratio, best, best_live, improved,
+                       frame_off, B, tab, tab_len, step, lr_clip, wd, H, nband, stride);
 }
 
 __global__ __launch_bounds__(256) void plateau_kernel(const float* __restrict__ loss, double* __restrict__ state,
diff --git a/aware_amd/runtime.py b/aware_amd/runtime.py
--- a/aware_amd/runtime.py
+++ b/aware_amd/runtime.py
@@ -232,6 +232,16 @@
     return mag, ph
 
 
+def polar_split(spec: torch.Tensor, unit_default: float = 1.0):
+    spec = spec.contiguous()
+    n = spec.numel() // 2
+    mag = torch.empty(spec.shape[:-1], dtype=torch.float32, device=spec.device)
+    unit = torch.empty_like(spec)
+    check(load_library().aware_polar_split(_ptr(spec), _ptr(mag), _ptr(unit), n, float(unit_default), _stream()),
+          "aware_polar_split")
+    return mag, unit
+
+
 def polar_decompose_bwd(spec, grad_mag, grad_phase):
     lib = load_library()
     gs = torch.empty_like(spec)
@@ -595,6 +605,19 @@
     def step(self):
         return self._view(8, (1,), torch.int32)
 
+    @property
+    def original_spectrum(self):
+        return self._view(14, (self.batch.total_frames, self.plan.band_stride, 2))
+
+    @property
+    def phasor(self):
+        return self._view(7, (self.batch.total_frames, self.plan.band_stride, 2))
+
+    @property
+    def moments(self):
+        return (self._view(15, (self.batch.total_frames, self.plan.band_stride)),
+                self._view(16, (self.batch.total_frames, self.plan.band_stride)))
+
     def clip_learning_rates(self) -> np.ndarray:
         if not self.lib.aware_embed_buffer(self.h, 11):
             raise AwareHipError("no optimiser was set with set_optimizer")
diff --git a/include/aware_hip.h b/include/aware_hip.h
--- a/include/aware_hip.h
+++ b/include/aware_hip.h
@@ -72,6 +72,7 @@
                     void* stream);
 
 int aware_polar_decompose(const void* spec, float* mag, float* phase, size_t n, void* stream);
+int aware_polar_split(const void* spec, float* mag, void* unit, size_t n, float unit_default, void* stream);
 int aware_polar_decompose_bwd(const void* spec, const float* grad_mag, const float* grad_phase, void* grad_spec, size_t n,
                               void* stream);
 int aware_polar_assemble(const float* mag, const float* phase, void* spec, size_t n, void* stream);
```

Result: no change. 1959 (median of 3 runs) (+0.4%).
